# refresh-bio/fqsqueezer

Measured on AMD Instinct MI355X. Metric: Mbases/s compressed (DNA stream, SE sorted), higher is better.
Workload: dtype u64; 1 GPU; 1000000x150bp SE, G=7500000 (seed 2+rank), -om s -gs 8 -qm n -im n; workers_T=64, blocks=256, per_gpu=one independent file per GPU

## Files before the change

fqsqueezer_amd/csrc/fqsx_api.hip:

```cpp
#include "fqsx_kernels.h"
#include "fqsx_qual.h"
#include "fqsx_qdec.h"
#include "../../include/fqsx.h"
#include "fqsx_vm.h"
#include "fqsx_rt.h"
#include <sys/resource.h>

#ifndef FQSX_EMU
#include <dlfcn.h>
#include <rccl/rccl.h>
#endif
#include <algorithm>
#include <cstdio>
#include <cstdlib>
#include <cstring>
#include <string>
#include <vector>

extern "C" const char *fqsx_last_error(void) { return g_err.c_str(); }
extern "C" const char *fqsx_version(void) {
#ifdef FQSX_EMU
  return "fqsx 0.1 (host emulation build - tests only)";
#else
  return "fqsx 0.1 (HIP gfx950)";
#endif
}

FQ_DEV bool phase_skip(const DevCfg &cfg) { return (cfg.err[0] | cfg.err[1]) != 0; }
FQ_KERNEL_NW(FQSX_INS_THREADS, FQSX_INS_WG_PER_CU * FQSX_INS_WAVES / 4) void k_insert_phase(DevCfg cfg, u64 nb_slots, u64 ns_slots, u32 win, u32 maxmult) {
  FQ_SHARED InsWgShared sm;
#ifndef FQSX_EMU
  if (FQ_TID == 0) sm.err = phase_skip(cfg) ? 1u : 0u;
  __syncthreads();
  const bool skip = sm.err != 0;
  __syncthreads();
  if (skip) return;
#else
  if (phase_skip(cfg)) return;
#endif
  if (FQ_BLOCK >= 3 * cfg.T) {
    const u64 stride = (u64)(FQ_NBLOCKS - 3 * cfg.T) * FQ_NTHREADS, first = (u64)(FQ_BLOCK - 3 * cfg.T) * FQ_NTHREADS + FQ_TID;
    for (u64 i = first; i < nb_slots; i += stride) cfg.l_b.slots[i] = 0;
    for (u64 i = first; i < ns_slots; i += stride) cfg.l_s.slots[i] = 0;
    for (u64 i = first; i < 2ull * cfg.T; i += stride) cfg.l_s.filled[i] = 0;
    return;
  }
  insert_phase_body(cfg, &sm, FQ_BLOCK / 3, FQ_BLOCK % 3, win, maxmult);
  if (cfg.sys_scope) fq_release_system();
}
FQ_KERNEL64 void k_compact_generic(const u8 *out, u64 out_cap, const u64 *lens, u8 *dst) {
  const u32 tid = FQ_BLOCK;
  u64 off = 0;
  for (u32 t = 0; t < tid; ++t) off += lens[t];
  const u64 n = lens[tid] <= out_cap ? lens[tid] : 0;
  const u8 *src = out + (u64)tid * out_cap;
  for (u64 i = FQ_LANE; i < n; i += FQ_WAVE) dst[off + i] = src[i];
}
FQ_KERNEL64 void k_clear_local(DevCfg cfg, u64 nb_slots, u64 ns_slots) {
  if (phase_skip(cfg)) return;
  const u64 stride = (u64)FQ_NBLOCKS * FQ_WAVE, first = (u64)FQ_BLOCK * FQ_WAVE + FQ_LANE;
  for (u64 i = first; i < nb_slots; i += stride) cfg.l_b.slots[i] = 0;
  for (u64 i = first; i < ns_slots; i += stride) cfg.l_s.slots[i] = 0;
  for (u64 i = first; i < 2ull * cfg.T; i += stride) cfg.l_s.filled[i] = 0;
}
FQ_KERNEL64 void k_finish_block(DevCfg cfg, u64 *lens , u64 *end ) {
  if (FQ_LANE == 0) {
    if (FQ_BLOCK == 0) { end[2 * cfg.T] = cfg.err[0]; end[2 * cfg.T + 1] = cfg.err[1]; }
    if (cfg.err[1]) return;
    finish_block_body(cfg, FQ_BLOCK);
    lens[FQ_BLOCK] = cfg.ws[FQ_BLOCK].out_len;
    end[FQ_BLOCK] = cfg.ws[FQ_BLOCK].out_len;
    end[cfg.T + FQ_BLOCK] = cfg.ctx_filled[FQ_BLOCK];
  }
}
FQ_KERNEL64 void k_gather_stats(DevCfg cfg, u64 *out) {
  for (u32 i = FQ_LANE; i < 64; i += FQ_WAVE) {
    u64 s = 0;
    for (u32 t = 0; t < cfg.T; ++t) s += cfg.ws[t].stat[i];
    out[i] = s;
  }
}
FQ_DEV void part_split(const DevCfg &cfg, u32 &kind, u32 &blk) {
  kind = 0;
  blk = FQ_BLOCK;
  for (; kind < 2; ++kind) {
    const u32 g = cfg.T * cfg.mail[kind].n_tiles;
    if (blk < g) break;
    blk -= g;
  }
}
FQ_KERNEL64 void k_part_count(DevCfg cfg) {
  FQ_SHARED u32 hist[256];
  u32 kind, blk;
  if (phase_skip(cfg)) return;
  part_split(cfg, kind, blk);
  part_count_body(cfg, kind, blk, hist);
}
FQ_KERNEL64 void k_part_scan(DevCfg cfg) {
  if (phase_skip(cfg)) return;
  part_scan_body(cfg, FQ_BLOCK / cfg.T, FQ_BLOCK % cfg.T);
}
FQ_DEV void part_dstoff_leader(const DevCfg &cfg, u32 kind, u32 *demand , u32 seg1);
FQ_KERNEL64 void k_part_dstoff(DevCfg cfg, u32 *demand , u32 seg1) {
  if (cfg.err[0] || (cfg.err[1] && cfg.err[1] != seg1)) {
    if (FQ_BLOCK == 0 && FQ_LANE == 0) demand[2 * cfg.T] = cfg.err[0];
    return;
  }
  part_dstoff_leader(cfg, FQ_BLOCK, demand, seg1);
}
FQ_DEV void part_dstoff_leader(const DevCfg &cfg, u32 kind, u32 *demand, u32 seg1) {
  part_dstoff_body(cfg, kind);
  if (kind != MAIL_P)
    for (u32 d = FQ_LANE; d < cfg.T; d += FQ_WAVE) {
      const u32 o = (kind == MAIL_S ? 0 : cfg.T) + d;
      demand[o] = cfg.mail[kind].dst_tot[d];
      demand[2 * cfg.T + 1 + o] = (kind == MAIL_S ? cfg.g_s : cfg.g_b).filled[d];
    }
  if (kind == 0 && FQ_LANE == 0) demand[2 * cfg.T] = *cfg.err;
  if (seg1 && kind != MAIL_P) {
    const KTab &t = kind == MAIL_S ? cfg.g_s : cfg.g_b;
    bool over = false;
    for (u32 d = FQ_LANE; d < cfg.T; d += FQ_WAVE) over |= ((u64)t.filled[d] + cfg.mail[kind].dst_tot[d]) * 100 > t.nb * FQSX_BKT * cfg.tab_load_pct;
    if (wave_any(over) && FQ_LANE == 0) cfg.err[1] = seg1;
  }
}
FQ_KERNEL64 void k_part_scatter(DevCfg cfg, u32 seg1, u32 *demand) {
  FQ_SHARED u32 cursor[256];
  FQ_SHARED u32 ld[64];
  FQ_SHARED u64 gm[256];
  FQ_SHARED u32 doff[257];
  u32 kind, blk;
  if (cfg.err[0] || (cfg.err[1] && cfg.err[1] != seg1)) return;
  part_split(cfg, kind, blk);
  if (demand) {
    const Mail &m = cfg.mail[kind];
    u32 run = 0;
    for (u32 base = 0; base < cfg.T; base += FQ_WAVE) {
      const u32 d = base + FQ_LANE;
      const u32 v = d < cfg.T ? m.dst_tot[d] : 0;
      const u32 ex = wave_excl_scan32(v) + run;
      if (d < cfg.T) doff[d] = ex;
      run += wave_sum32(v);
    }
    if (FQ_LANE == 0) doff[cfg.T] = run;
    FQ_SYNC();
    if (blk == 0) part_dstoff_leader(cfg, kind, demand, seg1);
  }
  part_scatter_body(cfg, kind, blk, cursor, ld, gm, demand ? doff : nullptr);
}
FQ_KERNEL64 void k_pe_demand(DevCfg cfg, u32 *demand, u32 seg1) {
  FQ_SHARED InsShared sm;
  if (seg1 && phase_skip(cfg)) return;
  pe_insert_body(cfg, &sm, FQ_BLOCK, true, demand);
  if (seg1 && FQ_LANE == 0 && ((u64)cfg.g_pe.filled[FQ_BLOCK] + demand[FQ_BLOCK]) * 2 > cfg.g_pe.cap_mask + 1) cfg.err[1] = seg1;
}
FQ_KERNEL void k_pe_bucket_count(DevCfg cfg) {
  if (phase_skip(cfg)) return;
  const u32 total = cfg.T * cfg.pe_cap, stride = FQ_GRID_STRIDE(u32);
  for (u32 g = FQ_GRID_FIRST(u32); g < total; g += stride) pe_bucket_count_body(cfg, g);
}
FQ_KERNEL64 void k_pe_bucket_offsets(DevCfg cfg, u32 seg1) {
  if (phase_skip(cfg)) return;
  u32 run = 0;
  bool over = false;
  for (u32 base = 0; base < cfg.T; base += FQ_WAVE) {
    const u32 o = base + FQ_LANE;
    const u32 v = o < cfg.T ? cfg.pe_bkt_n[o] : 0u;
    const u32 ex = wave_excl_scan32(v) + run;
    if (o < cfg.T) {
      cfg.pe_bkt_n[cfg.T + o] = ex;
      cfg.pe_bkt_cur[o] = 0;
      over |= ((u64)cfg.g_pe.filled[o] + v) * 2 > cfg.g_pe.cap_mask + 1;
    }
    run += wave_sum32(v);
  }
  if (FQ_LANE == 0) cfg.pe_bkt_n[2 * cfg.T] = run;
  if (wave_any(over) && FQ_LANE == 0) cfg.err[1] = seg1;
}
FQ_KERNEL void k_pe_bucket_scatter(DevCfg cfg) {
  if (phase_skip(cfg)) return;
  const u32 total = cfg.T * cfg.pe_cap, stride = FQ_GRID_STRIDE(u32);
  for (u32 g = FQ_GRID_FIRST(u32); g < total; g += stride) pe_bucket_scatter_body(cfg, g);
}
FQ_KERNEL64 void k_pe_insert_buckets(DevCfg cfg) {
  FQ_SHARED InsShared sm;
  if (phase_skip(cfg)) return;
  pe_insert_bucket_body(cfg, &sm, FQ_BLOCK);
  FQ_SYNC_MEM();
  if (FQ_LANE == 0) cfg.pe_bkt_n[FQ_BLOCK] = 0;
}
FQ_KERNEL64 void k_pe_insert(DevCfg cfg) {
  FQ_SHARED InsShared sm;
  if (phase_skip(cfg)) return;
  if (cfg.pe_part && FQ_BLOCK % cfg.shard_world != cfg.shard_rank) return;
  pe_insert_body(cfg, &sm, FQ_BLOCK, false, nullptr);
  if (cfg.sys_scope) fq_release_system();
}
FQ_KERNEL void k_rehash_ptab(PTab o, PTab n, u32 n_sub, u32 first, u32 step, u32 sys) {
  const u64 ocap = o.cap_mask + 1, total = ocap * n_sub;
  const u64 gstride = FQ_GRID_STRIDE(u64);
  for (u64 g = FQ_GRID_FIRST(u64); g < total; g += gstride) {
    const u32 sub = first + (u32)(g / ocap) * step;
    const u64 k = o.key[(u64)sub * o.stride + (g % ocap)], v = o.val[(u64)sub * o.stride + (g % ocap)];
    if (k == 0 && v == 0) continue;
    u64 *nk = n.key + (u64)sub * n.stride, *nv = n.val + (u64)sub * n.stride;
    u64 p = murmur64(k) & n.cap_mask;
    for (;;) {
      if (nk[p] == 0 && atomic_cas64(&nk[p], 0, k) == 0) { nv[p] = v; break; }
      p = (p + 1) & n.cap_mask;
    }
  }
  if (sys) fq_release_system();
}
FQ_KERNEL void k_zero_words(u64 *p, u64 n, u32 sys) {
  const u64 gstride = FQ_GRID_STRIDE(u64);
  for (u64 i = FQ_GRID_FIRST(u64); i < n; i += gstride) p[i] = 0;
  if (sys) fq_release_system();
}
FQ_KERNEL void k_rehash_ktab(KTab o, KTab n, u32 n_sub, u32 first, u32 step, u32 sys) {
  const u64 ocap = o.nb * FQSX_BKT;
  const u64 total = ocap * n_sub;
  const u64 gstride = FQ_GRID_STRIDE(u64);
  for (u64 g = FQ_GRID_FIRST(u64); g < total; g += gstride) {
    u32 sub = first + (u32)(g / ocap) * step;
    u64 it = o.slots[(u64)sub * o.stride + (g % ocap)];
    if (!it) continue;
    bool claimed = false;
    (void)tab_find_or_claim(n, n.slots + (u64)sub * n.stride, it >> n.cbits, it, claimed);
  }
  if (sys) fq_release_system();
}
FQ_KERNEL void k_rehash_ctx(const u64 *o, u64 ocap_mask, u64 *n, u64 ncap_mask, u32 T) {
  const u64 ocap = ocap_mask + 1, total = ocap * T;
  const u64 gstride = FQ_GRID_STRIDE(u64);
  for (u64 g = FQ_GRID_FIRST(u64); g < total; g += gstride) {
    u32 w = (u32)(g / ocap);
    const u64 *src = o + 4 * g;
    u64 q1 = src[1];
    u32 tag = slot_tag(q1);
    if (!tag) continue;
    u64 key = src[0];
    u64 *b = n + 4 * (u64)w * (ncap_mask + 1);
    u64 h = (u64)ctx_mix(tag, key) & ncap_mask;
    for (;;) {
      u64 *p = b + 4 * h;
      if (p[1] == 0 && atomic_cas64(&p[1], 0, q1) == 0) {
        p[0] = key; p[2] = src[2]; p[3] = src[3];
        break;
      }
      h = (h + 1) & ncap_mask;
    }
  }
}

FQ_KERNEL64 void k_shard_counts(DevCfg cfg, u32 *dst, u32 status) {
  const u32 T = cfg.T;
  if (FQ_BLOCK == 3 * T) {
    for (u32 s = FQ_LANE; s < T; s += FQ_WAVE) dst[3ull * T * T + s] = (cfg.pe_n && shard_mine(cfg, s)) ? cfg.pe_n[s] : 0u;
    if (FQ_LANE == 0) dst[3ull * T * T + T] = (status | cfg.err[0]) != 0 ? 1u : 0u;
    return;
  }
  const u32 kind = FQ_BLOCK / T, s = FQ_BLOCK % T;
  const Mail &m = cfg.mail[kind];
  for (u32 o = FQ_LANE; o < T; o += FQ_WAVE) {
    u32 n = 0;
    if (shard_mine(cfg, s))
      for (u32 t = 0; t < m.n_tiles; ++t) n += m.tile_hist[((u64)s * m.n_tiles + t) * T + cfg.vmap[o]];
    dst[((u64)kind * T + s) * T + o] = n;
  }
}
FQ_KERNEL void k_shard_colsum(DevCfg cfg, const u32 *C, u32 *cs) {
  const u32 T = cfg.T, G = cfg.shard_world;
  const u32 stride = FQ_GRID_STRIDE(u32), first = FQ_GRID_FIRST(u32);
  for (u32 i = first; i < 3 * T; i += stride) {
    const u32 kind = i / T, o = i % T;
    const u32 *Ck = C + (u64)kind * T * T;
    u32 tot = 0;
    for (u32 q = 0; q < G; ++q) {
      u32 n = 0;
      for (u32 s = q; s < T; s += 8 * G) {
        u32 v[8];
#pragma unroll
        for (u32 x = 0; x < 8; ++x) v[x] = s + x * G < T ? Ck[(u64)(s + x * G) * T + o] : 0u;
#pragma unroll
        for (u32 x = 0; x < 8; ++x) n += v[x];
      }
      cs[((u64)kind * (G + 1) + 1 + q) * T + o] = n;
      tot += n;
    }
    cs[((u64)kind * (G + 1)) * T + o] = tot;
  }
}
FQ_KERNEL64 void k_shard_need(DevCfg cfg, const u32 *cs, u64 *out, u64 *stats_before) {
  const u32 T = cfg.T;
  for (u32 which = 0; which < 2; ++which) {
    const KTab &t = which ? cfg.g_b : cfg.g_s;
    const u32 *tot = cs + (u64)(which ? MAIL_B : MAIL_S) * (cfg.shard_world + 1) * T;
    u64 need = 0;
    for (u32 o = FQ_LANE; o < T; o += FQ_WAVE) {
      const u64 n = (u64)t.filled[o] + tot[o];
      need = n > need ? n : need;
// ... 88 lines not shown
    if (o == T - 1) m.dst_off[T] = dst + tot;
  }
  if (o % G != me) return;
  u32 run = 0;
  for (u32 sb = 0; sb < T; sb += FQ_WAVE) {
    const u32 s = sb + FQ_LANE;
    const u32 v = s < T ? Ck[(u64)s * T + o] : 0u;
    const u32 ex = wave_excl_scan32(v) + run;
    if (s < T) { col[s] = v; pre[s] = ex; }
    run += wave_sum32(v);
  }
  FQ_SYNC();
  u32 chunk0 = 0;
  for (u32 q = 0; q < G; ++q) {
    u32 before = 0, size = 0;
    for (u32 jb = 0; jb < n_own; jb += FQ_WAVE) {
      const u32 j = jb + FQ_LANE, o2 = me + j * G;
      u32 n = 0;
      if (j < n_own) {
        if (cs) n = cs[((u64)kind * (G + 1) + 1 + q) * T + o2];
        else for (u32 s = q; s < T; s += G) n += Ck[(u64)s * T + o2];
      }
      before += wave_sum32(j < n_own && o2 < o ? n : 0u);
      size += wave_sum32(j < n_own ? n : 0u);
    }
    u32 src = chunk0 + before;
    for (u32 s = q; s < T; s += G) {
      if (FQ_LANE == 0) soff[s] = src;
      src += col[s];
    }
    chunk0 += size;
  }
  FQ_SYNC();
  for (u32 x = FQ_LANE; x < tot; x += FQ_WAVE) {
    u32 lo = 0, hi = T;
    while (hi - lo > 1) {
      const u32 mid = (lo + hi) >> 1;
      if (pre[mid] <= x) lo = mid; else hi = mid;
    }
    while (col[lo] == 0 && lo > 0) --lo;
    m.sorted[dst + x] = recv[soff[lo] + (x - pre[lo])];
  }
}
FQ_KERNEL void k_shard_collect(DevCfg cfg, u32 kind, u64 *out) {
  const Mail &m = cfg.mail[kind];
  const u32 total = m.dst_off[cfg.T];
  const u32 stride = FQ_GRID_STRIDE(u32), first = FQ_GRID_FIRST(u32);
  for (u32 e = first; e < total; e += stride) {
    const u64 x = m.sorted[e];
    if (kind == MAIL_P) { out[e] = (x << 2) | siv_test(&cfg, x); continue; }
    const KTab &t = kind == MAIL_S ? cfg.g_s : cfg.g_b;
    const u64 *sl = t.slots + (u64)sb_owner(&cfg, x) * t.stride;
    const u64 item = tab_locate(t, sl, x >> (64 - 2 * t.k)).item;
    out[e] = item;
  }
}
FQ_KERNEL void k_shard_apply(DevCfg cfg, u32 kind, const u64 *items, u32 n) {
  const u32 stride = FQ_GRID_STRIDE(u32), first = FQ_GRID_FIRST(u32);
  for (u32 e = first; e < n; e += stride) {
    const u64 item = items[e];
    if (kind == MAIL_P && cfg.siv_part) {
      if (item) siv_idx_move(cfg, item >> 4, (u32)((item >> 2) & 3), (u32)(item & 3));
      continue;
    }
    if (kind == MAIL_P) {
      const u64 idx = item >> 2, val = item & 3;
      u64 *wp = cfg.siv + (idx >> 5);
      const u32 sh = 2 * (u32)(idx & 31);
      u64 old = *wp;
      for (;;) {
        if (((old >> sh) & 3) >= val) break;
        const u64 seen = atomic_cas64(wp, old, (old & ~(3ull << sh)) | (val << sh));
        if (seen == old) { siv_idx_move(cfg, idx, (u32)((old >> sh) & 3), (u32)val); break; }
        old = seen;
      }
      continue;
    }
    if (!item) continue;
    const KTab &t = kind == MAIL_S ? cfg.g_s : cfg.g_b;
    const u64 v = item >> t.cbits;
    const u32 sub = sb_owner(&cfg, v << (64 - 2 * t.k));
    bool claimed = false;
    u64 *slot = tab_find_or_claim(t, t.slots + (u64)sub * t.stride, v, item, claimed);
    if (!slot) continue;
    if (claimed) {
      atomic_add32(&t.filled[sub], 1u);
      continue;
    }
    u64 old = *(volatile u64 *)slot;
    while ((old & ((1ull << t.cbits) - 1ull)) < (item & ((1ull << t.cbits) - 1ull))) {
      const u64 seen = atomic_cas64(slot, old, item);
      if (seen == old) break;
      old = seen;
    }
  }
}

struct fqsx_dna : DevCtx {
  DevCfg cfg;
  u32 T;
  u64 gs_cap, gb_cap, ls_cap, lb_cap, ctx_cap, gpe_cap, lpe_cap;
  u32 pe_bkt_cap;
  bool paired;
  u32 mail_cap[3];
  u64 dev_bases_cap, dev_off_cap;
  u8 *d_bases;
  u64 *d_off;
  u32 *d_demand;
  u64 *d_lens;
  u8 *d_compact;
  u64 compact_cap, din_cap, dout_cap;
  std::vector<u32> h_demand, h_filled;
  std::vector<u8> h_out;
  std::vector<u64> h_lens;
  u32 n_growths;
  u32 tab_small_pct;
  u32 tab_load_pct, tab_after_pct;
  u8 *h_pin;
  u64 *d_end;
  bool filled_valid;
  u32 cur_n_reads, cur_S, cur_gen;
  u64 cur_need_lb, cur_need_ls, cur_need_lpe;
  bool cur_decode;
  u32 shard_rank, shard_world = 1;
  u8 *d_vmap;
  u64 *d_xbuf;
  u64 xbuf_cap;
  u32 *d_cglob;
  u32 *d_colsum;
  u64 siv_before[2];
  fqsx_comm comm;
  bool comm_set, shard_apply_own;
  u64 *d_xrecv[3];
  u64 xrecv_cap[3];
  u64 *d_items, *d_gathered, *d_small;
  u64 items_cap, gathered_cap;
  std::vector<u32> h_cglob;
  u64 sh_phases, sh_collectives, sh_a2a_words, sh_gather_words;
  bool part;
  bool part_fallback;
  u64 vm_gran;
  fqsx_vm::FdMesh mesh;
  struct VmTab {
    u8 *va = nullptr;
    u64 va_bytes = 0, chunk_bytes = 0;
    std::vector<fqsx_vm::Handle> h;
    std::vector<u8> mapped;
    u64 own_bytes = 0;
    u32 own_mod = 0;
    bool live = false;
  } vm_s, vm_b, vm_pk, vm_pv, vm_siv;
  u32 *d_plog_n;
  u32 ins_win, ins_maxmult;
  u64 vm_own_bytes;
};

namespace {

#define FQSX_PIN_BYTES (64u * 1024u)
int d2h_small_begin(fqsx_dna *c, const void *d, u64 bytes) { return d2h(c, c->h_pin, d, bytes); }
int d2h_small_end(fqsx_dna *c, void *h, u64 bytes) {
  DEVCHK(dev_sync(c));
  memcpy(h, c->h_pin, bytes);
  return FQSX_OK;
}

#define REHASH_GRID FQ_GRID(2048)

int collect_streams(DevCtx *c, u8 *d_compact, u32 T, const u8 *d_out, u64 out_cap, const u64 *d_lens,
                    const std::vector<u64> &lens_host, std::vector<u8> &h_out, const u8 **streams, u64 *lens) {
  int rc;
  u64 total = 0;
  for (u32 t = 0; t < T; ++t) total += lens_host[t];
  h_out.resize(total ? total : 1);
  if (total) {
    LAUNCH(c, 2, k_compact_generic, T, 64, d_out, out_cap, d_lens, d_compact);
    if ((rc = d2h_sync(c, h_out.data(), d_compact, total))) return rc;
  }
  u64 pos = 0;
  for (u32 t = 0; t < T; ++t) {
    streams[t] = h_out.data() + pos;
    lens[t] = lens_host[t];
    pos += lens_host[t];
  }
  return FQSX_OK;
}

u64 pow2_at_least(u64 x) {
  u64 p = 1;
  while (p < x) p <<= 1;
  return p;
}

bool tab_over(const fqsx_dna *c, u64 need, u64 cap) { return need * 100 > cap * c->tab_load_pct; }
u64 tab_new_cap(const fqsx_dna *c, u64 need) {
  const u32 after = need * c->T * sizeof(u64) * 100 / 40 < (256ull << 20) ? std::min<u32>(c->tab_small_pct, c->tab_after_pct) : c->tab_after_pct;
  u64 cap = (need * 100 + after - 1) / after + 2 * FQSX_BKT;
  return (cap + FQSX_BKT - 1) / FQSX_BKT * FQSX_BKT;
}

KGeom make_geom(u32 k) {
  KGeom g;
  g.k = k;
  g.shift = 64 - 2 * k;
  g.mask = (~0ull) << g.shift;
  g.kernel_mask = ((1ull << (2 * k - 8)) - 1ull) << (64 - 2 * k + 4);
  return g;
}

void mt_seed(u32 *s, u32 seed) {
  s[0] = seed;
  for (int i = 1; i < 624; ++i) s[i] = 1812433253u * (s[i - 1] ^ (s[i - 1] >> 30)) + (u32)i;
}

int ktab_alloc(fqsx_dna *c, KTab &t, u32 n_sub, u64 cap, u32 k, u32 cbits, bool with_filled) {
  void *p = nullptr;
  int rc = dalloc(c, &p, cap * n_sub * sizeof(u64), true);
  if (rc) return rc;
  t.slots = (u64 *)p;
  t.nb = cap / FQSX_BKT;
  t.stride = cap;
  t.k = k;
  t.cbits = cbits;
  if (with_filled) {
    rc = dalloc(c, &p, (u64)n_sub * sizeof(u32), true);
    if (rc) return rc;
    t.filled = (u32 *)p;
  }
  return FQSX_OK;
}

#define VMCHK(x) do { std::string e_; if (g_vm_dbg) fprintf(stderr, "[fqsx vm] %s\n", #x); if ((x)) { g_err = "partitioned tables: " + e_; return FQSX_E_HIP; } } while (0)
static const bool g_vm_dbg = getenv("FQSX_VM_DEBUG") != nullptr;
u32 vt_rank(const fqsx_dna *c, const fqsx_dna::VmTab &v, u32 o) { return (v.own_mod ? o % v.own_mod : o) % c->shard_world; }
void vtab_drop(fqsx_dna *c, fqsx_dna::VmTab &v, u32 o) {
  if (!v.live || !v.mapped[o]) return;
  std::string e;
  (void)fqsx_vm::unmap(v.va + (u64)o * v.chunk_bytes, v.chunk_bytes, e);
  (void)fqsx_vm::release(v.h[o], e);
  v.mapped[o] = 0;
  if (vt_rank(c, v, o) == c->shard_rank) { c->dev_bytes -= v.chunk_bytes; c->vm_own_bytes -= v.chunk_bytes; v.own_bytes -= v.chunk_bytes; }
}
void vtab_free(fqsx_dna *c, fqsx_dna::VmTab &v) {
  if (!v.live) return;
  std::string e;
  for (u32 o = 0; o < (u32)v.h.size(); ++o) vtab_drop(c, v, o);
#ifdef FQSX_EMU
  (void)fqsx_vm::unreserve(v.va, v.va_bytes, e);
#else
#endif
  v = fqsx_dna::VmTab();
}
u64 vm_min_chunk(const fqsx_dna *c) {
#ifndef FQSX_EMU
  return std::max<u64>(c->vm_gran, 2ull << 20);
#else
  return c->vm_gran;
#endif
}
int vtab_reserve_raw(fqsx_dna *c, fqsx_dna::VmTab &v, u64 cap, u64 *stride_out, u32 n_chunks = 0) {
  const u32 T = n_chunks ? n_chunks : c->T;
  const u64 min_chunk = vm_min_chunk(c);
  const u64 gran_slots = min_chunk / sizeof(u64);
  const u64 stride = (cap + gran_slots - 1) / gran_slots * gran_slots;
  v = fqsx_dna::VmTab();
  v.chunk_bytes = stride * sizeof(u64);
  v.va_bytes = v.chunk_bytes * T;
  v.h.assign(T, fqsx_vm::Handle());
  v.mapped.assign(T, 0);
  VMCHK(fqsx_vm::reserve(v.va_bytes, std::max<u64>(c->vm_gran, std::min<u64>(v.chunk_bytes, 2ull << 20)), &v.va, e_));
  v.live = true;
  *stride_out = stride;
  return FQSX_OK;
}
int vtab_reserve(fqsx_dna *c, KTab &t, fqsx_dna::VmTab &v, u64 cap, u32 k, u32 cbits) {
  u64 stride = 0;
  const int rc = vtab_reserve_raw(c, v, cap, &stride);
  if (rc) return rc;
  t.slots = (u64 *)v.va;
  t.nb = cap / FQSX_BKT;
  t.stride = stride;
  t.k = k;
  t.cbits = cbits;
  return FQSX_OK;
}
int vtab_create_own(fqsx_dna *c, fqsx_dna::VmTab &v, u32 o) {
  VMCHK(fqsx_vm::create(c->device, v.chunk_bytes, &v.h[o], e_));
  c->dev_bytes += v.chunk_bytes; c->vm_own_bytes += v.chunk_bytes; v.own_bytes += v.chunk_bytes;
  c->dev_bytes_peak = std::max(c->dev_bytes_peak, c->dev_bytes);
  VMCHK(fqsx_vm::map(c->device, v.va + (u64)o * v.chunk_bytes, v.chunk_bytes, v.h[o], e_));
  v.mapped[o] = 1;
  const u64 words = v.chunk_bytes / sizeof(u64);
  LAUNCH(c, 2, k_zero_words, (u32)std::min<u64>(REHASH_GRID, (words + 255) / 256), 256, (u64 *)(v.va + (u64)o * v.chunk_bytes), words, c->cfg.sys_scope);
  return FQSX_OK;
}
int vtab_exchange(fqsx_dna *c, fqsx_dna::VmTab &v) {
  const u32 T = (u32)v.h.size(), G = c->shard_world, me = c->shard_rank;
  if (G == 1) return FQSX_OK;
  std::vector<std::vector<u32>> of(G);
  for (u32 o = 0; o < T; ++o) of[vt_rank(c, v, o)].push_back(o);
  size_t longest = 0;
  for (u32 q = 0; q < G; ++q) longest = std::max(longest, of[q].size());
  const size_t R = 128;
  for (size_t r0 = 0; r0 < longest; r0 += R) {
    std::vector<int> mine;
    for (size_t j = r0; j < std::min(of[me].size(), r0 + R); ++j) {
// ... 158 lines not shown
  c->n_growths += 1;
  return FQSX_OK;
}

int grow_ctx(fqsx_dna *c, u64 new_cap) {
  void *p = nullptr;
  int rc = dalloc(c, &p, new_cap * c->T * sizeof(CtxSlot), true);
  if (rc) return rc;
  LAUNCH(c, 2, k_rehash_ctx, REHASH_GRID, 256, (const u64 *)c->cfg.ctx, c->cfg.ctx_cap_mask, (u64 *)p, new_cap - 1, c->T);
  DEVCHK(dev_sync(c));
  dfree(c, c->cfg.ctx);
  c->cfg.ctx = (CtxSlot *)p;
  c->cfg.ctx_cap_mask = new_cap - 1;
  c->ctx_cap = new_cap;
  return FQSX_OK;
}

int mail_alloc(fqsx_dna *c, u32 kind, u32 cap) {
  Mail &m = c->cfg.mail[kind];
  const u32 T = c->T;
  dfree(c, m.list); dfree(c, m.sorted); dfree(c, m.tile_hist);
  m.list = m.sorted = nullptr; m.tile_hist = nullptr;
  m.cap = m.n_tiles = 0; c->mail_cap[kind] = 0;
  cap = (cap + FQSX_TILE - 1) / FQSX_TILE * FQSX_TILE;
  void *p = nullptr;
  int rc;
  if ((rc = dalloc(c, &p, (u64)T * cap * sizeof(u64), false))) return rc;
  m.list = (u64 *)p;
  if ((rc = dalloc(c, &p, (u64)T * cap * sizeof(u64), false))) return rc;
  m.sorted = (u64 *)p;
  m.cap = cap;
  m.n_tiles = cap / FQSX_TILE;
  if ((rc = dalloc(c, &p, (u64)T * m.n_tiles * T * sizeof(u32), false))) return rc;
  m.tile_hist = (u32 *)p;
  c->mail_cap[kind] = cap;
  return FQSX_OK;
}

int launch_segment(fqsx_dna *c, bool decode, u32 n_reads, u32 S, u32 seg) {
  EncArgs a;
  a.cfg = c->cfg;
  a.n_reads = n_reads; a.S = S; a.seg = seg; a.pad = (u32)c->k_n[0];
  return dev_launch(c, 0, true, [&] {
    return decode ? fqsx_launch_decode(c->stream, a) : c->paired ? fqsx_launch_encode_pe(c->stream, a) : fqsx_launch_encode_se(c->stream, a);
  });
}

int block_prepare(fqsx_dna *c, const u8 *d_bases, const u64 *d_off, const u64 *h_off, u32 n_reads, u32 generation,
                  const u8 *const *dec_streams = nullptr, const u64 *dec_lens = nullptr) {
  const bool decode = dec_streams != nullptr;
  const u32 T = c->T;
  DevCfg &cfg = c->cfg;
  u64 S = generation < 100u ? 100u - generation : 0u;
  u64 cap_s = (u64)n_reads / T / 2;
  if (S > cap_s) S = cap_s;
  if (S) --S;
  u64 max_wbases = 0, max_seg_bases = 0, max_seg_reads = 0, max_wreads = 0;
  std::vector<u64> wbases(T);
  for (u32 t = 0; t < T; ++t) {
    u64 first, last;
    worker_reads(t, T, n_reads, first, last);
    wbases[t] = h_off[last] - h_off[first];
    max_wbases = std::max(max_wbases, wbases[t]);
    max_wreads = std::max(max_wreads, last - first);
    u64 cur = first;
    for (u64 seg = 0; seg <= S; ++seg) {
      u64 stop = last;
      if (seg < S) {
        const u64 ns = segment_synchro(seg, S, first, last);
        if (!c->paired) stop = ns + 1;
        else { u64 i = cur; if (i < ns) i += (ns - i + 1) & ~1ull; stop = i + 2; }
      }
      if (stop > last) stop = last;
      if (stop > cur) {
        max_seg_bases = std::max(max_seg_bases, h_off[stop] - h_off[cur]);
        max_seg_reads = std::max(max_seg_reads, stop - cur);
        cur = stop;
      }
    }
  }
  int rc;
  void *p = nullptr;
  if (c->paired && (n_reads & 1)) { g_err = "paired-end blocks need an even number of reads"; return FQSX_E_ARG; }
  u64 need_out = max_wbases + 16 * max_wreads + 1024;
  if ((rc = dfit(c, cfg.out, cfg.out_cap, need_out, pow2_at_least(need_out), T))) return rc;
  const u64 mail_entries[3] = {2 * max_seg_bases + 2 * max_seg_reads, max_seg_bases, 2 * max_seg_bases};
  for (u32 k = 0; k < 3; ++k) {
    u64 need = mail_entries[k] + 64;
    if (need > c->mail_cap[k] && (rc = mail_alloc(c, k, (u32)(need + need / 4)))) return rc;
  }
  u64 need_lb = pow2_at_least(4 * max_seg_bases + 64), need_ls = pow2_at_least(2 * max_seg_bases + 64);
  if ((rc = ltab_fit(c, cfg.l_b, c->lb_cap, need_lb, cfg.bmer, 6))) return rc;
  if ((rc = ltab_fit(c, cfg.l_s, c->ls_cap, need_ls, cfg.smer, 12))) return rc;
  u64 need_lpe = 0;
  if (c->paired) {
    const u64 seg_pairs = max_seg_reads / 2 + 1;
    const u64 need_list = 14 * seg_pairs + 16;
    const u32 list_cap = (u32)(need_list + need_list / 4);
    if ((rc = dfit(c, cfg.pe_bkt, c->pe_bkt_cap, need_list, list_cap, (u64)T * 3 * sizeof(u64)))) return rc;
    if ((rc = dfit(c, cfg.pe_list, cfg.pe_cap, need_list, list_cap, (u64)T * 3 * sizeof(u64)))) return rc;
    need_lpe = pow2_at_least(2 * 14 * seg_pairs + 64);
    if ((rc = lpe_fit(c, cfg.l_pe, c->lpe_cap, need_lpe))) return rc;
    cfg.l_pe.cap_mask = need_lpe - 1;
    cfg.l_pe.stride = need_lpe;
    u64 max_len = 0;
    for (u32 i = 0; i < n_reads; ++i) max_len = std::max(max_len, h_off[i + 1] - h_off[i]);
    if (!decode && max_len > FQSX_RD_LDS && (rc = dfit(c, cfg.pe_scr, cfg.pe_scr_cap, max_len + 128, (max_len + max_len / 4 + 128 + 63) & ~63ull, (u64)T * 3, true))) return rc;
  }
  cfg.l_b.nb = need_lb / FQSX_BKT; cfg.l_b.stride = need_lb;
  cfg.l_s.nb = need_ls / FQSX_BKT; cfg.l_s.stride = need_ls;
  if (!c->filled_valid && (rc = d2h_sync(c, c->h_filled.data(), cfg.ctx_filled, T * sizeof(u32)))) return rc;
  c->filled_valid = false;
  {
    u64 need = 0;
    for (u32 t = 0; t < T; ++t) need = std::max<u64>(need, (u64)c->h_filled[t] + 2 * wbases[t] + 64);
#ifdef FQSX_TIMING
    if (generation % 64 == 63) fprintf(stderr, "[timing] block %u: ctx slots used by worker 0: %u, capacity %llu\n", generation, c->h_filled[0], (unsigned long long)c->ctx_cap);
#endif
    if (need * 2 > c->ctx_cap && (rc = grow_ctx(c, pow2_at_least(need * 2)))) return rc;
  }
  cfg.bases = d_bases;
  cfg.read_off = d_off;
  if (decode) {
    std::vector<u64> doff(T + 1, 0);
    for (u32 t = 0; t < T; ++t) doff[t + 1] = doff[t] + dec_lens[t];
    u64 max_len = 0;
    for (u32 i = 0; i < n_reads; ++i) max_len = std::max(max_len, h_off[i + 1] - h_off[i]);
    const u64 need_in = doff[T] + 64, need_out = h_off[n_reads] + 64, need_sc = max_len + 64;
    if ((rc = dfit(c, cfg.din, c->din_cap, need_in, need_in + need_in / 4, 1))) return rc;
    if ((rc = dfit(c, cfg.dout, c->dout_cap, need_out, need_out + need_out / 4, 1))) return rc;
    if ((rc = dfit(c, cfg.dscratch, cfg.dcap, need_sc, need_sc + need_sc / 4, (u64)T * 2))) return rc;
    if (!cfg.din_off && (rc = dalloc(c, &p, ((u64)T + 1) * sizeof(u64), false))) return rc;
    if (!cfg.din_off) cfg.din_off = (const u64 *)p;
    std::vector<u8> flat(doff[T] ? doff[T] : 1);
    for (u32 t = 0; t < T; ++t) memcpy(flat.data() + doff[t], dec_streams[t], dec_lens[t]);
    if ((rc = h2d(c, (void *)cfg.din, flat.data(), doff[T]))) return rc;
    if ((rc = h2d(c, (void *)cfg.din_off, doff.data(), (T + 1) * sizeof(u64)))) return rc;
    DEVCHK(dev_sync(c));
  }

  c->cur_n_reads = n_reads; c->cur_S = (u32)S; c->cur_gen = generation;
  c->cur_need_lb = need_lb; c->cur_need_ls = need_ls; c->cur_need_lpe = need_lpe;
  c->cur_decode = decode;
  return FQSX_OK;
}

int clear_local_tables(fqsx_dna *c) {
  const u64 words = (c->cur_need_lb + c->cur_need_ls) * c->T;
  const u32 grid = (u32)std::min<u64>(2048, (words + 4095) / 4096 + 1);
  LAUNCH(c, 2, k_clear_local, grid, 64, c->cfg, c->cur_need_lb * c->T, c->cur_need_ls * c->T);
  return FQSX_OK;
}

int insert_and_clear(fqsx_dna *c) {
  const u64 words = (c->cur_need_lb + c->cur_need_ls) * c->T;
  const u64 per = 64ull * FQSX_INS_THREADS;
  const u32 cgrid = (u32)std::min<u64>(2048, (words + per - 1) / per + 1);
  LAUNCH(c, 1, k_insert_phase, 3 * c->T + cgrid, FQSX_INS_THREADS, c->cfg, c->cur_need_lb * c->T, c->cur_need_ls * c->T, c->ins_win, c->ins_maxmult);
  return FQSX_OK;
}
int grow_for_demand(fqsx_dna *c) {
  const u32 T = c->T;
  DevCfg &cfg = c->cfg;
  int rc;
  for (int which = 0; which < 2; ++which) {
    KTab &t = which ? cfg.g_b : cfg.g_s;
    u64 &cap = which ? c->gb_cap : c->gs_cap;
    u64 need = 0;
    for (u32 o = 0; o < T; ++o) need = std::max<u64>(need, (u64)c->h_demand[2 * T + 1 + which * T + o] + c->h_demand[which * T + o]);
    if (tab_over(c, need, cap) && (rc = grow_global(c, t, cap, tab_new_cap(c, need)))) return rc;
  }
  return FQSX_OK;
}
int pe_insert_and_clear(fqsx_dna *c);
int pe_clear_local(fqsx_dna *c);
int block_recover(fqsx_dna *c, u32 seg) {
  const u32 T = c->T;
  int rc;
  if ((rc = d2h_sync(c, c->h_demand.data(), c->d_demand, (4 * T + 1) * sizeof(u32)))) return rc;
  const u64 before = c->gs_cap + c->gb_cap + c->gpe_cap;
  if ((rc = grow_for_demand(c))) return rc;
  if ((rc = dzero(c, c->cfg.err + 1, sizeof(u32)))) return rc;
  if (c->paired) {
    if ((rc = dzero(c, c->cfg.pe_bkt_n, T * sizeof(u32)))) return rc;
    LAUNCH(c, 2, k_pe_demand, T, 64, c->cfg, c->d_demand + 4 * T + 1, 0u);
    std::vector<u32> dem(T), fil(T);
    if ((rc = d2h_sync(c, dem.data(), c->d_demand + 4 * T + 1, T * sizeof(u32)))) return rc;
    if ((rc = d2h_sync(c, fil.data(), c->cfg.g_pe.filled, T * sizeof(u32)))) return rc;
    u64 need = 0;
    for (u32 o = 0; o < T; ++o) need = std::max<u64>(need, (u64)fil[o] + dem[o]);
    if (need * 2 > c->gpe_cap && (rc = grow_gpe(c, pow2_at_least(need * 2 + 2)))) return rc;
  }
  if (c->gs_cap + c->gb_cap + c->gpe_cap == before) { g_err = "phase " + std::to_string(seg) + " posted for growth, but no table needs it"; return FQSX_E_DEVICE; }
  if (c->paired && (rc = pe_insert_and_clear(c))) return rc;
  return insert_and_clear(c);
}
int pe_clear_local(fqsx_dna *c) {
  const u32 T = c->T;
  DevCfg &cfg = c->cfg;
  int rc;
  if ((rc = dzero(c, cfg.l_pe.key, c->cur_need_lpe * T * sizeof(u64)))) return rc;
  if ((rc = dzero(c, cfg.l_pe.val, c->cur_need_lpe * T * sizeof(u64)))) return rc;
  return dzero(c, cfg.l_pe.filled, T * sizeof(u32));
}
int pe_insert_and_clear(fqsx_dna *c) {
  LAUNCH(c, 2, k_pe_insert, c->T, 64, c->cfg);
  return pe_clear_local(c);
}

int block_segment(fqsx_dna *c, u32 seg) {
  const u32 T = c->T, n_reads = c->cur_n_reads;
  const u64 S = c->cur_S, need_lpe = c->cur_need_lpe;
  const bool decode = c->cur_decode;
  DevCfg &cfg = c->cfg;
  int rc;
  {
    if ((rc = launch_segment(c, decode, n_reads, (u32)S, seg))) return rc;
    const u32 part_grid = T * (cfg.mail[0].n_tiles + cfg.mail[1].n_tiles + cfg.mail[2].n_tiles);
    LAUNCH(c, 2, k_part_count, part_grid, 64, cfg);
    LAUNCH(c, 2, k_part_scan, 3 * T, 64, cfg);
    if (!decode) {
      LAUNCH(c, 2, k_part_scatter, part_grid, 64, cfg, seg + 1, c->d_demand);
      if (c->paired) {
        const u32 bgrid = FQ_GRID((u32)std::min<u64>(1024, ((u64)T * cfg.pe_cap + 255) / 256));
        LAUNCH(c, 2, k_pe_bucket_count, bgrid, 256, cfg);
        LAUNCH(c, 2, k_pe_bucket_offsets, 1, 64, cfg, seg + 1);
        LAUNCH(c, 2, k_pe_bucket_scatter, bgrid, 256, cfg);
        LAUNCH(c, 2, k_pe_insert_buckets, T, 64, cfg);
        if ((rc = pe_clear_local(c))) return rc;
      }
      return insert_and_clear(c);
    }
    LAUNCH(c, 2, k_part_dstoff, 3, 64, cfg, c->d_demand, 0u);
    if ((rc = d2h_small_begin(c, c->d_demand, (4 * T + 1) * sizeof(u32)))) return rc;
    LAUNCH(c, 2, k_part_scatter, part_grid, 64, cfg, 0u, (u32 *)nullptr);
    if ((rc = d2h_small_end(c, c->h_demand.data(), (4 * T + 1) * sizeof(u32)))) return rc;
    if (c->h_demand[2 * T]) {
      g_err = "device error " + std::to_string(c->h_demand[2 * T]) + " in encode kernel";
      return FQSX_E_DEVICE;
    }
    if ((rc = grow_for_demand(c))) return rc;
    if (c->paired) {
      LAUNCH(c, 2, k_pe_demand, T, 64, cfg, c->d_demand, 0u);
      if ((rc = d2h_sync(c, c->h_demand.data(), c->d_demand, T * sizeof(u32)))) return rc;
      if ((rc = d2h_sync(c, c->h_filled.data(), cfg.g_pe.filled, T * sizeof(u32)))) return rc;
      u64 need = 0;
      for (u32 o = 0; o < T; ++o) need = std::max<u64>(need, (u64)c->h_filled[o] + c->h_demand[o]);
      if (need * 2 > c->gpe_cap && (rc = grow_gpe(c, pow2_at_least(need * 2 + 2)))) return rc;
      if ((rc = pe_insert_and_clear(c))) return rc;
    }
    LAUNCH(c, 1, k_insert_phase, 3 * T, FQSX_INS_THREADS, cfg, (u64)0, (u64)0, c->ins_win, c->ins_maxmult);
    if ((rc = clear_local_tables(c))) return rc;
  }
  return FQSX_OK;
}

int block_finish(fqsx_dna *c, const u64 *h_off, const u8 **streams, u64 *lens, u8 *bases_out, u32 *posted = nullptr) {
  if (posted) *posted = 0;
  const u32 T = c->T, n_reads = c->cur_n_reads, generation = c->cur_gen;
  const bool decode = c->cur_decode;
  DevCfg &cfg = c->cfg;
  int rc;
  if (decode) {
    u32 derr = 0;
    if ((rc = d2h_sync(c, &derr, cfg.err, sizeof(u32)))) return rc;
    if (derr) {
      g_err = "device error " + std::to_string(derr) + " while decoding block " + std::to_string(generation);
      return FQSX_E_DEVICE;
    }
    return bases_out ? d2h_sync(c, bases_out, cfg.dout, h_off[n_reads]) : FQSX_OK;
  }
  LAUNCH(c, 2, k_finish_block, T, 64, cfg, c->d_lens, c->d_end);
  {
    std::vector<u64> e(2 * T + 2);
    if ((rc = d2h_small_begin(c, c->d_end, e.size() * sizeof(u64)))) return rc;
    if ((rc = d2h_small_end(c, e.data(), e.size() * sizeof(u64)))) return rc;
    if (e[2 * T]) {
      g_err = "device error " + std::to_string(e[2 * T]) + " while encoding block " + std::to_string(generation);
      return FQSX_E_DEVICE;
    }
    if (e[2 * T + 1]) {
      if (posted) { *posted = (u32)e[2 * T + 1]; return FQSX_OK; }
      g_err = "growth posted by the device outside the deferred path";
      return FQSX_E_DEVICE;
    }
    for (u32 t = 0; t < T; ++t) { c->h_lens[t] = e[t]; c->h_filled[t] = (u32)e[T + t]; }
    c->filled_valid = true;
  }
  u64 total = 0;
  for (u32 t = 0; t < T; ++t) {
    if (c->h_lens[t] > cfg.out_cap) { g_err = "stream overflow"; return FQSX_E_DEVICE; }
    total += c->h_lens[t];
  }
  if ((rc = dfit(c, c->d_compact, c->compact_cap, total, total + total / 2 + 4096, 1))) return rc;
  return collect_streams(c, c->d_compact, T, cfg.out, cfg.out_cap, c->d_lens, c->h_lens, c->h_out, streams, lens);
}

int encode_block_impl(fqsx_dna *c, const u8 *d_bases, const u64 *d_off, const u64 *h_off, u32 n_reads, u32 generation,
                      const u8 **streams, u64 *lens, const u8 *const *dec_streams = nullptr, const u64 *dec_lens = nullptr,
                      u8 *bases_out = nullptr) {
  if (c->shard_world > 1) { g_err = "a sharded codec is driven through fqsx_shard_* (fqsqueezer_amd/sharded.py)"; return FQSX_E_ARG; }
  int rc = block_prepare(c, d_bases, d_off, h_off, n_reads, generation, dec_streams, dec_lens);
  for (u32 seg = 0; !rc;) {
    for (; !rc && seg <= c->cur_S; ++seg) rc = block_segment(c, seg);
    u32 posted = 0;
    if (!rc) rc = block_finish(c, h_off, streams, lens, bases_out, &posted);
    if (rc || !posted) break;
    rc = block_recover(c, posted - 1);
    seg = posted;
  }
  return rc;
}

int create_impl(fqsx_dna *c, const u8 *h) {
  const u32 T = c->T;
  DevCfg &cfg = c->cfg;
  memset(&cfg, 0, sizeof(cfg));
  cfg.T = T;
  cfg.mode = h[5];
  cfg.prefix = h[10]; cfg.pmer = h[11]; cfg.smer = h[12]; cfg.bmer = h[13];
  cfg.gp = make_geom(cfg.pmer); cfg.gs = make_geom(cfg.smer); cfg.gb = make_geom(cfg.bmer);
  cfg.pmer_mod_shift = 2 * cfg.pmer - 12;
  cfg.T_magic = ((1ull << 32) + T - 1) / T;
  cfg.T_pow2 = (T & (T - 1)) == 0 ? 1u : 0u;
  cfg.dbg = 0;
  if (const char *e = getenv("FQSX_PROTO_DEBUG")) cfg.dbg = (u32)strtoul(e, nullptr, 0);
  cfg.ps_nobytes_n = (2 * cfg.pmer + 7) / 8;
  int rc;
  void *p = nullptr;
  if ((rc = dalloc(c, &p, (1ull << (2 * cfg.pmer)) / 4, true))) return rc;
  cfg.siv = (u64 *)p;
  if ((rc = dalloc(c, &p, 2 * sizeof(u64), true))) return rc;
  cfg.siv_stats = (u64 *)p;
  if ((rc = dalloc(c, &p, ((1ull << (2 * cfg.pmer)) >> FQSX_SIV_BLK_LOG) * 4 * sizeof(u32), true))) return rc;
  cfg.siv_idx = (u32 *)p;
  c->tab_load_pct = 80; c->tab_after_pct = 62;
  if (const char *e = getenv("FQSX_TAB_LOAD_PCT")) c->tab_load_pct = (u32)std::min<u64>(85, std::max<u64>(20, strtoull(e, nullptr, 10)));
  c->tab_small_pct = 40;
  if (const char *e = getenv("FQSX_TAB_AFTER_PCT")) c->tab_small_pct = c->tab_after_pct = (u32)std::min<u64>(c->tab_load_pct - 5, std::max<u64>(10, strtoull(e, nullptr, 10)));
  cfg.tab_load_pct = c->tab_load_pct;
  c->ins_win = FQSX_WIN_MAX; c->ins_maxmult = 16;
  if (const char *e = getenv("FQSX_INS_WINDOW")) c->ins_win = (u32)std::min<u64>(FQSX_WIN_MAX, std::max<u64>(1, strtoull(e, nullptr, 10)));
  if (const char *e = getenv("FQSX_INS_MAXMULT")) c->ins_maxmult = (u32)std::min<u64>(FQSX_WIN_MULT_MAX, std::max<u64>(1, strtoull(e, nullptr, 10)));
  if (const char *e = getenv("FQSX_INS_PARALLEL")) if (atoi(e) == 0) c->ins_win = 0;
#ifdef FQSX_EMU
  c->ins_win = 0;
#endif
  if (const char *e = getenv("FQSX_WHATIF")) { u32 r = 0, u = 0; if (sscanf(e, "%u,%u", &r, &u) == 2) cfg.whatif = (r << 16) | (u & 0xffffu); }
  c->gs_cap = c->gb_cap = pow2_at_least(std::max<u64>(1024, (1ull << 22) / T));
  if (const char *e = getenv("FQSX_GTAB_INIT")) c->gs_cap = c->gb_cap = pow2_at_least(std::max<u64>(64, strtoull(e, nullptr, 10)));
  if ((rc = ktab_alloc(c, cfg.g_s, T, c->gs_cap, cfg.smer, 12, true))) return rc;
  if ((rc = ktab_alloc(c, cfg.g_b, T, c->gb_cap, cfg.bmer, 6, true))) return rc;
  cfg.g_s.two = cfg.g_b.two = 1;
  c->ls_cap = c->lb_cap = 1024;
  if ((rc = ktab_alloc(c, cfg.l_s, T, c->ls_cap, cfg.smer, 12, false))) return rc;
  if ((rc = ktab_alloc(c, cfg.l_b, T, c->lb_cap, cfg.bmer, 6, false))) return rc;
  if ((rc = dalloc(c, &p, 2 * (u64)T * sizeof(u32), true))) return rc;
  cfg.l_s.filled = (u32 *)p;
  cfg.l_b.filled = (u32 *)p + T;
  c->ctx_cap = 1u << 14;
  if ((rc = dalloc(c, &p, c->ctx_cap * T * sizeof(CtxSlot), true))) return rc;
  cfg.ctx = (CtxSlot *)p;
  cfg.ctx_cap_mask = c->ctx_cap - 1;
  if ((rc = dalloc(c, &p, T * sizeof(u32), true))) return rc;
  cfg.ctx_filled = (u32 *)p;
  {
    std::vector<u16> tpl(SM_OFF_BYTE, 0);
    auto fill = [&](u32 off, u32 entries, u32 stride, u32 n) {
      for (u32 e = 0; e < entries; ++e) {
        for (u32 i = 0; i < n; ++i) tpl[off + e * stride + i] = 1;
        tpl[off + e * stride + n] = (u16)n;
      }
    };
    fill(SM_OFF_FLAGS, 256, SM_FLAGS_N + 1, SM_FLAGS_N);
    fill(SM_OFF_NS, 32, SM_NS_N + 1, SM_NS_N);
    fill(SM_OFF_PSF, 65536, SM_PSF_N + 1, SM_PSF_N);
    fill(SM_OFF_PSNB, 65536, 6, cfg.ps_nobytes_n);
    fill(SM_OFF_NIB, 68, SM_NIB_N + 1, SM_NIB_N);
    tpl.resize(SM_TOTAL_U16, 0);
    fill(SM_OFF_MID, 1, SM_NIB_N + 1, SM_NIB_N);
    if ((rc = dalloc(c, &p, (u64)T * SM_TOTAL_U16 * sizeof(u16), false))) return rc;
    cfg.small = (u16 *)p;
    if ((rc = h2d(c, cfg.small, tpl.data(), tpl.size() * sizeof(u16)))) return rc;
    DEVCHK(dev_sync(c));
    for (u32 t = 1; t < T; ++t)
      if ((rc = d2d(c, cfg.small + (u64)t * SM_TOTAL_U16, cfg.small, tpl.size() * sizeof(u16)))) return rc;
    if ((rc = dalloc(c, &p, (u64)T * SM_LAZY_ENTRIES, true))) return rc;
    cfg.byte_init = (u8 *)p;
  }
  {
    std::vector<WState> ws(1);
    memset(ws.data(), 0, sizeof(WState));
    for (int g = 0; g < 4; ++g) {
      mt_seed(ws[0].mt[g], 5481);
      ws[0].mt_idx[g] = 624;
    }
    if ((rc = dalloc(c, &p, (u64)T * sizeof(WState), false))) return rc;
    cfg.ws = (WState *)p;
    for (u32 t = 0; t < T; ++t)
      if ((rc = h2d(c, cfg.ws + t, ws.data(), sizeof(WState)))) return rc;
    DEVCHK(dev_sync(c));
  }
  for (u32 k = 0; k < 3; ++k) {
    if ((rc = dalloc(c, &p, (u64)T * sizeof(u32), true))) return rc;
    cfg.mail[k].n = (u32 *)p;
    if ((rc = dalloc(c, &p, (u64)T * sizeof(u32), true))) return rc;
    cfg.mail[k].dst_tot = (u32 *)p;
    if ((rc = dalloc(c, &p, ((u64)T + 1) * sizeof(u32), true))) return rc;
    cfg.mail[k].dst_off = (u32 *)p;
    if ((rc = mail_alloc(c, k, FQSX_TILE))) return rc;
  }
  c->paired = cfg.mode >= 2;
  c->gpe_cap = c->lpe_cap = 0;
  if (c->paired) {
    c->gpe_cap = pow2_at_least(std::max<u64>(1024, (1ull << 20) / T));
    if (const char *e = getenv("FQSX_PTAB_INIT")) c->gpe_cap = pow2_at_least(std::max<u64>(64, strtoull(e, nullptr, 10)));
    if ((rc = ptab_alloc(c, cfg.g_pe, T, c->gpe_cap, true))) return rc;
    c->lpe_cap = 1024;
    if ((rc = ptab_alloc(c, cfg.l_pe, T, c->lpe_cap, true))) return rc;
    if ((rc = dalloc(c, &p, (u64)T * sizeof(u32), true))) return rc;
    cfg.pe_n = (u32 *)p;
    if ((rc = dalloc(c, &p, (3 * (u64)T + 1) * sizeof(u32), true))) return rc;
    cfg.pe_bkt_n = (u32 *)p;
    cfg.pe_bkt_cur = cfg.pe_bkt_n + 2 * T + 1;
  }
  {
    u8 ident[256];
    for (u32 i = 0; i < 256; ++i) ident[i] = (u8)i;
    if ((rc = dalloc(c, &p, 256, false))) return rc;
    c->d_vmap = (u8 *)p;
    cfg.vmap = c->d_vmap;
    if ((rc = h2d(c, c->d_vmap, ident, 256))) return rc;
    DEVCHK(dev_sync(c));
  }
  cfg.shard_rank = 0; cfg.shard_world = 1; cfg.shard_cnt = nullptr;
  if ((rc = dalloc(c, &p, sizeof(u32) * 4, true))) return rc;
  cfg.err = (u32 *)p;
#ifdef FQSX_TIMING
  if ((rc = dalloc(c, &p, (u64)FQSX_TRACE_LAUNCHES * T * FQSX_TRACE_W * sizeof(u64), true))) return rc;
  cfg.trace = (u64 *)p;
#endif
  if ((rc = dalloc(c, &p, (5 * (u64)T + 2) * sizeof(u32), true))) return rc;
  c->d_demand = (u32 *)p;
  if ((rc = dalloc(c, &p, ((u64)T + 64) * sizeof(u64), true))) return rc;
  c->d_lens = (u64 *)p;
  if ((rc = dalloc(c, &p, (2 * (u64)T + 2) * sizeof(u64), true))) return rc;
  c->d_end = (u64 *)p;
  if ((rc = pinned_alloc((void **)&c->h_pin, FQSX_PIN_BYTES))) return rc;
  c->h_demand.assign(4 * T + 1, 0);
  c->h_filled.assign(T, 0);
  c->h_lens.assign(T + 64, 0);
  DEVCHK(dev_sync(c));
  return FQSX_OK;
}

}

extern "C" {

int fqsx_dna_create(const uint8_t *h, int device, fqsx_dna **out) { return fqsx_dna_create_on_partition(h, device, 0, 1, out); }

int fqsx_dna_create_on_partition(const uint8_t *h, int device, uint32_t part, uint32_t n_parts, fqsx_dna **out) {
  if (n_parts == 0 || part >= n_parts) { g_err = "bad compute-unit partition"; return FQSX_E_ARG; }
  if (!h || !out || h[0] != 'K' || h[1] != 'C' || h[2] != 'S' || h[3] != 'D') {
    g_err = "malformed .fqs parameter header";
    return FQSX_E_ARG;
  }
  if (h[4] == 0) { g_err = "no_threads must be >= 1"; return FQSX_E_ARG; }
  if (h[5] > 3) { g_err = "unknown dna_mode"; return FQSX_E_ARG; }
  if (h[11] < 12 || h[11] > 18 || h[12] <= h[11] || h[13] <= h[12] + 1 || h[13] > 27 || h[10] >= h[11]) {
    g_err = "unsupported k-mer lengths";
    return FQSX_E_ARG;
  }
  fqsx_dna *c = new fqsx_dna();
  c->T = h[4];
  int rc = dev_open(c, device, part, n_parts);
  if (rc) {
    delete c;
    return rc;
  }
  rc = create_impl(c, h);
  if (!rc && getenv("FQSX_CHUNKED_TABLES") && atoi(getenv("FQSX_CHUNKED_TABLES"))) rc = fqsx_dna_use_chunked_tables(c);
  if (rc) {
    fqsx_dna_destroy(c);
    return rc;
  }
  *out = c;
  return FQSX_OK;
}

void fqsx_dna_destroy(fqsx_dna *c) {
  if (!c) return;
  dev_close(c);
  vtab_free(c, c->vm_s);
  vtab_free(c, c->vm_b);
  vtab_free(c, c->vm_pk);
  vtab_free(c, c->vm_pv);
  vtab_free(c, c->vm_siv);
  fqsx_vm::mesh_close(c->mesh);
  pinned_free(c->h_pin);
  delete c;
}

int fqsx_dna_encode_block_dev(fqsx_dna *c, const uint8_t *d_bases, const uint64_t *d_off, const uint64_t *h_off,
                              uint32_t n_reads, uint32_t generation, const uint8_t **streams, uint64_t *lens) {
  if (!c || !d_bases || !d_off || !h_off || !streams || !lens) { g_err = "null argument"; return FQSX_E_ARG; }
  DEVCHK(dev_enter(c));
  return encode_block_impl(c, d_bases, d_off, h_off, n_reads, generation, streams, lens);
}

int fqsx_dna_encode_block(fqsx_dna *c, const uint8_t *bases, const uint64_t *off, uint32_t n_reads, uint32_t generation,
                          const uint8_t **streams, uint64_t *lens) {
  if (!c || !bases || !off || !streams || !lens) { g_err = "null argument"; return FQSX_E_ARG; }
  DEVCHK(dev_enter(c));
  int rc;
  u64 nb = off[n_reads] + 64, no = ((u64)n_reads + 1) * sizeof(u64);
  if ((rc = dfit(c, c->d_bases, c->dev_bases_cap, nb, nb + nb / 4, 1))) return rc;
  if ((rc = dfit(c, c->d_off, c->dev_off_cap, no, no + no / 4, 1))) return rc;
  if ((rc = h2d(c, c->d_bases, bases, off[n_reads]))) return rc;
  if ((rc = h2d(c, c->d_off, off, no))) return rc;
  return encode_block_impl(c, c->d_bases, c->d_off, off, n_reads, generation, streams, lens);
}

int fqsx_dna_decode_block(fqsx_dna *c, const uint8_t *const *streams, const uint64_t *lens, const uint64_t *off, uint32_t n_reads,
                          uint32_t generation, uint8_t *bases_out) {
  if (!c || !streams || !lens || !off || !bases_out) { g_err = "null argument"; return FQSX_E_ARG; }
  DEVCHK(dev_enter(c));
  int rc;
  u64 no = ((u64)n_reads + 1) * sizeof(u64);
  if ((rc = dfit(c, c->d_off, c->dev_off_cap, no, no + no / 4, 1))) return rc;
  if ((rc = h2d(c, c->d_off, off, no))) return rc;
  return encode_block_impl(c, nullptr, c->d_off, off, n_reads, generation, nullptr, nullptr, streams, lens, bases_out);
}

int fqsx_dna_decode_block_dev(fqsx_dna *c, const uint8_t *const *streams, const uint64_t *lens, const uint64_t *off, uint32_t n_reads,
                              uint32_t generation, const uint8_t **d_bases_out) {
  if (d_bases_out) *d_bases_out = nullptr;
  if (!c || !streams || !lens || !off || !d_bases_out) { g_err = "null argument"; return FQSX_E_ARG; }
  DEVCHK(dev_enter(c));
  int rc;
  u64 no = ((u64)n_reads + 1) * sizeof(u64);
  if ((rc = dfit(c, c->d_off, c->dev_off_cap, no, no + no / 4, 1))) return rc;
  if ((rc = h2d(c, c->d_off, off, no))) return rc;
  if ((rc = encode_block_impl(c, nullptr, c->d_off, off, n_reads, generation, nullptr, nullptr, streams, lens, nullptr))) return rc;
  *d_bases_out = c->cfg.dout;
  return FQSX_OK;
}

int fqsx_shard_config(fqsx_dna *c, uint32_t rank, uint32_t world) {
  if (!c || world == 0 || rank >= world || world > c->T) { g_err = "bad rank / world size"; return FQSX_E_ARG; }
  if (c->part && world > 1) { g_err = "a codec with chunked tables cannot be sharded afterwards (fqsx_shard_partition_tables after the attach)"; return FQSX_E_ARG; }
  DEVCHK(dev_enter(c));
  const u32 T = c->T;
  c->shard_rank = rank; c->shard_world = world;
  c->cfg.shard_rank = rank; c->cfg.shard_world = world;
  u8 vm[256];
  for (u32 i = 0; i < 256; ++i) vm[i] = (u8)i;
  u32 v = 0;
  for (u32 q = 0; q < world; ++q)
    for (u32 o = q; o < T; o += world) vm[o] = (u8)v++;
  int rc;
  void *p = nullptr;
  if ((rc = h2d(c, c->d_vmap, vm, 256))) return rc;
  if (!c->cfg.shard_cnt) {
    if ((rc = dalloc(c, &p, (3ull * T * T + T + 1) * sizeof(u32), true))) return rc;
    c->cfg.shard_cnt = (u32 *)p;
    if ((rc = dalloc(c, &p, (3ull * T * T + T + 1) * sizeof(u32), true))) return rc;
    c->d_cglob = (u32 *)p;
    if ((rc = dalloc(c, &p, 3ull * (T + 1) * T * sizeof(u32), true))) return rc;
    c->d_colsum = (u32 *)p;
    if ((rc = dalloc(c, &p, 8 * sizeof(u64), true))) return rc;
    c->d_small = (u64 *)p;
    c->h_cglob.assign(3ull * T * T + T + 1, 0);
  }
  DEVCHK(dev_sync(c));
  return FQSX_OK;
}

int fqsx_shard_begin_block(fqsx_dna *c, const uint8_t *bases , const uint64_t *off , const uint64_t *h_off,
                           uint32_t n_reads, uint32_t generation, uint32_t *n_segments) {
  if (!c || !bases || !off || !h_off || !n_segments) { g_err = "null argument"; return FQSX_E_ARG; }
  if (c->part) { g_err = "partitioned tables are driven through fqsx_shard_encode_block"; return FQSX_E_ARG; }
  if (c->paired && c->shard_world > 1) { g_err = "paired-end files are sharded through fqsx_shard_attach + fqsx_shard_encode_block (the step-wise fqsx_shard_* driver does not exchange the pair-table triples)"; return FQSX_E_ARG; }
  DEVCHK(dev_enter(c));
  int rc = block_prepare(c, bases, off, h_off, n_reads, generation);
  *n_segments = c->cur_S + 1;
  return rc;
}

int fqsx_shard_encode(fqsx_dna *c, uint32_t seg, uint32_t *counts ) {
  if (!c || !counts) { g_err = "null argument"; return FQSX_E_ARG; }
  DEVCHK(dev_enter(c));
  const u32 T = c->T;
  DevCfg &cfg = c->cfg;
  int rc;
  if ((rc = launch_segment(c, false, c->cur_n_reads, c->cur_S, seg))) return rc;
  const u32 part_grid = T * (cfg.mail[0].n_tiles + cfg.mail[1].n_tiles + cfg.mail[2].n_tiles);
  LAUNCH(c, 2, k_part_count, part_grid, 64, cfg);
  LAUNCH(c, 2, k_shard_counts, 3 * T + 1, 64, cfg, cfg.shard_cnt, 0u);
  if ((rc = d2d(c, counts, cfg.shard_cnt, 3ull * T * T * sizeof(u32)))) return rc;
  u32 err = 0;
  if ((rc = d2h_sync(c, &err, cfg.err, sizeof(u32)))) return rc;
  if (err) { g_err = "device error " + std::to_string(err) + " in encode kernel"; return FQSX_E_DEVICE; }
  return FQSX_OK;
}

int fqsx_shard_pack(fqsx_dna *c, const uint32_t *counts_sum , uint64_t *const send[3] ) {
  if (!c || !counts_sum || !send) { g_err = "null argument"; return FQSX_E_ARG; }
  DEVCHK(dev_enter(c));
  const u32 T = c->T;
  DevCfg &cfg = c->cfg;
  int rc;
  if ((rc = d2d(c, c->d_cglob, counts_sum, 3ull * T * T * sizeof(u32)))) return rc;
  const u32 part_grid = T * (cfg.mail[0].n_tiles + cfg.mail[1].n_tiles + cfg.mail[2].n_tiles);
  LAUNCH(c, 2, k_part_scan, 3 * T, 64, cfg);
  LAUNCH(c, 2, k_part_dstoff, 3, 64, cfg, c->d_demand, 0u);
  LAUNCH(c, 2, k_part_scatter, part_grid, 64, cfg, 0u, (u32 *)nullptr);
  std::vector<u32> tot(3 * (T + 1));
  for (u32 k = 0; k < 3; ++k)
    if ((rc = d2h_sync(c, tot.data() + k * (T + 1), cfg.mail[k].dst_off, (T + 1) * sizeof(u32)))) return rc;
  for (u32 k = 0; k < 3; ++k) {
    const u64 n = tot[k * (T + 1) + T];
    if (n && (rc = d2d(c, send[k], cfg.mail[k].sorted, n * sizeof(u64)))) return rc;
  }
  DEVCHK(dev_sync(c));
  return FQSX_OK;
}

int fqsx_shard_merge(fqsx_dna *c, const uint64_t *const recv[3] , uint64_t need[2]) {
  if (!c || !recv || !need) { g_err = "null argument"; return FQSX_E_ARG; }
  DEVCHK(dev_enter(c));
  const u32 T = c->T;
  DevCfg &cfg = c->cfg;
  int rc;
  for (u32 k = 0; k < 3; ++k) LAUNCH(c, 2, k_shard_merge, T, 64, cfg, k, recv[k], (const u32 *)c->d_cglob);
  need[0] = need[1] = 0;
  std::vector<u32> tot(T), fil(T);
  for (int which = 0; which < 2; ++which) {
    const KTab &t = which ? cfg.g_b : cfg.g_s;
    if ((rc = d2h_sync(c, tot.data(), cfg.mail[which ? MAIL_B : MAIL_S].dst_tot, T * sizeof(u32)))) return rc;
    if ((rc = d2h_sync(c, fil.data(), t.filled, T * sizeof(u32)))) return rc;
    for (u32 o = 0; o < T; ++o) need[which] = std::max<u64>(need[which], (u64)tot[o] + fil[o]);
  }
  return FQSX_OK;
}

int fqsx_shard_insert(fqsx_dna *c, uint64_t need_s, uint64_t need_b, uint64_t *const items[3] , uint64_t siv_delta[2]) {
  if (!c || !items || !siv_delta) { g_err = "null argument"; return FQSX_E_ARG; }
  DEVCHK(dev_enter(c));
  const u32 T = c->T;
  DevCfg &cfg = c->cfg;
  int rc;
  if (tab_over(c, need_s, c->gs_cap) && (rc = grow_global(c, cfg.g_s, c->gs_cap, tab_new_cap(c, need_s)))) return rc;
  if (tab_over(c, need_b, c->gb_cap) && (rc = grow_global(c, cfg.g_b, c->gb_cap, tab_new_cap(c, need_b)))) return rc;
  if ((rc = d2h_sync(c, c->siv_before, cfg.siv_stats, 2 * sizeof(u64)))) return rc;
  LAUNCH(c, 1, k_insert_phase, 3 * T, FQSX_INS_THREADS, cfg, (u64)0, (u64)0, c->ins_win, c->ins_maxmult);
  u64 after[2];
  if ((rc = d2h_sync(c, after, cfg.siv_stats, 2 * sizeof(u64)))) return rc;
  siv_delta[0] = after[0] - c->siv_before[0];
  siv_delta[1] = after[1] - c->siv_before[1];
  for (u32 k = 0; k < 3; ++k) LAUNCH(c, 2, k_shard_collect, REHASH_GRID, 256, cfg, k, items[k]);
  DEVCHK(dev_sync(c));
  return FQSX_OK;
}

int fqsx_shard_apply(fqsx_dna *c, uint32_t kind, const uint64_t *items , uint64_t n) {
  if (!c || kind > 2 || (!items && n)) { g_err = "bad argument"; return FQSX_E_ARG; }
  DEVCHK(dev_enter(c));
  if (n) LAUNCH(c, 2, k_shard_apply, REHASH_GRID, 256, c->cfg, kind, items, (u32)n);
  return FQSX_OK;
}

int fqsx_shard_end_phase(fqsx_dna *c, const uint64_t siv_delta_sum[2]) {
  if (!c || !siv_delta_sum) { g_err = "null argument"; return FQSX_E_ARG; }
  DEVCHK(dev_enter(c));
  int rc;
  u64 now[2] = {c->siv_before[0] + siv_delta_sum[0], c->siv_before[1] + siv_delta_sum[1]};
  if ((rc = h2d(c, c->cfg.siv_stats, now, 2 * sizeof(u64)))) return rc;
  DEVCHK(dev_sync(c));
  return clear_local_tables(c);
}

int fqsx_shard_finish_block(fqsx_dna *c, const uint64_t *h_off, const uint8_t **streams, uint64_t *lens) {
  if (!c || !h_off || !streams || !lens) { g_err = "null argument"; return FQSX_E_ARG; }
  DEVCHK(dev_enter(c));
  return block_finish(c, h_off, streams, lens, nullptr);
}

namespace {
int xbuf_fit(fqsx_dna *c, u64 *&buf, u64 &cap, u64 words) { return dfit(c, buf, cap, words, words + words / 4 + 1024, sizeof(u64)); }
#define COMMCHK(x, what) do { if ((x) != 0) { if (g_err.empty() || g_err.find(what) == std::string::npos) g_err = std::string(what) + " failed"; if (c->comm.abort) c->comm.abort(c->comm.ctx); return FQSX_E_HIP; } } while (0)

int shard_vote(fqsx_dna *c, int fail, const char *what) {
  const u64 NC = 3ull * c->T * c->T + c->T + 1;
  u32 *word = c->d_cglob + NC - 1;
  u32 v = fail ? 1u : 0u;
  const std::string mine = g_err;
  int rc;
  if ((rc = h2d(c, word, &v, sizeof(v)))) return rc;
  DEVCHK(dev_sync(c));
  COMMCHK(c->comm.allreduce_sum_u32(c->comm.ctx, word, 1), "all-reduce of the phase's status vote");
  if ((rc = d2h_sync(c, &v, word, sizeof(v)))) return rc;
  c->sh_collectives += 1;
  if (fail) { g_err = mine; return fail; }
  if (v) { g_err = std::string("another rank of the world failed in ") + what + " (this rank was fine): the phase is given up on every rank"; return FQSX_E_PEER; }
  return FQSX_OK;
}

int shard_phase_native(fqsx_dna *c, u32 seg) {
  const u32 T = c->T, G = c->shard_world, me = c->shard_rank;
  DevCfg &cfg = c->cfg;
  const u64 NC = 3ull * T * T + T + 1;
  int rc;
  if ((rc = launch_segment(c, false, c->cur_n_reads, c->cur_S, seg))) return rc;
  const u32 part_grid = T * (cfg.mail[0].n_tiles + cfg.mail[1].n_tiles + cfg.mail[2].n_tiles);
  LAUNCH(c, 2, k_part_count, part_grid, 64, cfg);
  LAUNCH(c, 2, k_shard_counts, 3 * T + 1, 64, cfg, c->d_cglob, 0u);
  COMMCHK(c->comm.allreduce_sum_u32(c->comm.ctx, c->d_cglob, NC), "all-reduce of the mailbox counts");
  LAUNCH(c, 2, k_shard_colsum, (3 * T + 63) / 64, 64, cfg, (const u32 *)c->d_cglob, c->d_colsum);
  LAUNCH(c, 2, k_shard_need, 1, 64, cfg, (const u32 *)c->d_colsum, c->d_small + 2, c->d_small);
  u64 small[3];
  if ((rc = d2h(c, c->h_cglob.data(), c->d_cglob, NC * sizeof(u32)))) return rc;
  if ((rc = d2h_sync(c, small, c->d_small + 2, sizeof(small)))) return rc;
  const u32 *C = c->h_cglob.data();
  if (C[NC - 1]) {
    if (small[2]) { g_err = "device error " + std::to_string(small[2]) + " in encode kernel"; return FQSX_E_DEVICE; }
    g_err = "device error in the encode kernel of another rank of the world (this rank was fine): the phase is given up on every rank";
    return FQSX_E_PEER;
  }
  std::vector<u64> vol(3ull * G * G, 0);
  for (u32 k = 0; k < 3; ++k)
    for (u32 s = 0; s < T; ++s)
      for (u32 o = 0; o < T; ++o) vol[((u64)k * G + s % G) * G + o % G] += C[((u64)k * T + s) * T + o];
  LAUNCH(c, 2, k_part_scan, 3 * T, 64, cfg);
  LAUNCH(c, 2, k_part_dstoff, 3, 64, cfg, c->d_demand, 0u);
  LAUNCH(c, 2, k_part_scatter, part_grid, 64, cfg, 0u, (u32 *)nullptr);
  std::vector<u64> sc(3ull * G), rcnt(3ull * G);
  const u64 *send[3];
  u64 *recv[3];
  u64 recv_need[3] = {0, 0, 0};
  for (u32 k = 0; k < 3; ++k) {
    for (u32 q = 0; q < G; ++q) {
      sc[(u64)k * G + q] = vol[((u64)k * G + me) * G + q];
      rcnt[(u64)k * G + q] = vol[((u64)k * G + q) * G + me];
      if (q != me) c->sh_a2a_words += sc[(u64)k * G + q];
      u64 n_in = 0;
      for (u32 f = 0; f < G; ++f) n_in += vol[((u64)k * G + f) * G + q];
      recv_need[k] = std::max(recv_need[k], n_in + 1);
    }
  }
  u64 M[3] = {0, 0, 0}, PM = 0;
  std::vector<u64> n_items(3ull * G, 0), pe_tot(G, 0);
  for (u32 k = 0; k < 3; ++k)
    for (u32 q = 0; q < G; ++q) {
      if (c->part && k != MAIL_P) continue;
      if (G == 1 && !c->shard_apply_own) continue;
      for (u32 f = 0; f < G; ++f) n_items[(u64)k * G + q] += vol[((u64)k * G + f) * G + q];
      M[k] = std::max(M[k], n_items[(u64)k * G + q]);
    }
  const u32 n_own_max = (T + G - 1) / G;
  const u32 n_fill = c->part ? (cfg.pe_part ? 3u : 2u) : 0u;
  const u64 FW = (u64)n_fill * n_own_max;
  if (c->paired)
    for (u32 s = 0; s < T; ++s) { pe_tot[s % G] += C[3ull * T * T + s]; PM = std::max(PM, pe_tot[s % G]); }
  const u64 off_k[3] = {0, M[0], M[0] + M[1]}, off_siv = M[0] + M[1] + M[2], off_fill = off_siv + 2, off_pe = off_fill + FW, W = off_pe + 3 * PM;
  const bool grow_s = tab_over(c, small[0], c->gs_cap), grow_b = tab_over(c, small[1], c->gb_cap);
  int inj_rank = -1, inj_phase = -1;
  if (const char *e = getenv("FQSX_TEST_FAIL")) (void)sscanf(e, "%d,%d", &inj_rank, &inj_phase);
  const bool injected = inj_phase >= 0 && (u64)inj_phase == c->sh_phases;
  if (injected || grow_s || grow_b || W > c->items_cap || W * G > c->gathered_cap || recv_need[0] > c->xrecv_cap[0] || recv_need[1] > c->xrecv_cap[1] ||
      recv_need[2] > c->xrecv_cap[2]) {
    int fail = 0;
    if (injected && (u32)inj_rank == me) { fail = FQSX_E_NOMEM; g_err = "injected allocation failure (FQSX_TEST_FAIL)"; }
    for (u32 k = 0; k < 3 && !fail; ++k) fail = xbuf_fit(c, c->d_xrecv[k], c->xrecv_cap[k], recv_need[k]);
    if (!fail) fail = xbuf_fit(c, c->d_items, c->items_cap, W);
    if (!fail) fail = xbuf_fit(c, c->d_gathered, c->gathered_cap, W * G);
    if (!fail && grow_s) fail = grow_global(c, cfg.g_s, c->gs_cap, tab_new_cap(c, small[0]));
    if (!fail && grow_b) fail = grow_global(c, cfg.g_b, c->gb_cap, tab_new_cap(c, small[1]));
    if (fail && c->part) fqsx_vm::mesh_close(c->mesh);
    if ((rc = shard_vote(c, fail, "the allocations / table growth of a phase"))) return rc;
  }
  for (u32 k = 0; k < 3; ++k) { send[k] = cfg.mail[k].sorted; recv[k] = c->d_xrecv[k]; }
  COMMCHK(c->comm.alltoallv_u64(c->comm.ctx, 3, send, sc.data(), recv, rcnt.data()), "all-to-all of the mailboxes");
  LAUNCH(c, 2, k_shard_merge3, 3 * T, 64, cfg, (const u64 *)c->d_xrecv[0], (const u64 *)c->d_xrecv[1], (const u64 *)c->d_xrecv[2], (const u32 *)c->d_cglob, (const u32 *)c->d_colsum);
  if (cfg.siv_part) {
    cfg.p_log = c->d_items + off_k[MAIL_P];
    if (M[MAIL_P]) LAUNCH(c, 2, k_zero_words, (u32)std::min<u64>(REHASH_GRID, (M[MAIL_P] + 255) / 256), 256, cfg.p_log, M[MAIL_P], 0u);
    if ((rc = dzero(c, c->d_plog_n, sizeof(u32)))) return rc;
  }
  LAUNCH(c, 1, k_insert_phase, 3 * T, FQSX_INS_THREADS, cfg, (u64)0, (u64)0, c->ins_win, c->ins_maxmult);
  for (u32 k = 0; k < 3; ++k)
    if (n_items[(u64)k * G + me] && !(k == MAIL_P && cfg.siv_part)) LAUNCH(c, 2, k_shard_collect, REHASH_GRID, 256, cfg, k, c->d_items + off_k[k]);
  if (FW) LAUNCH(c, 2, k_shard_pack2, 1, 64, cfg, (const u64 *)c->d_small, c->d_items + off_siv, c->d_items + off_fill, n_own_max, n_fill);
  else LAUNCH(c, 2, k_shard_siv_delta, 1, 64, cfg, (const u64 *)c->d_small, c->d_items + off_siv);
  if (c->paired && PM) LAUNCH(c, 2, k_shard_pe_pack, T, 64, cfg, c->d_items + off_pe);
  COMMCHK(c->comm.allgather_u64(c->comm.ctx, c->d_items, W, c->d_gathered), "all-gather of the applied items");
  c->sh_gather_words += W * (G - 1);
  for (u32 q = 0; q < G; ++q)
    if (q != me || c->shard_apply_own)
      for (u32 k = 0; k < 3; ++k)
        if (n_items[(u64)k * G + q] && !(k == MAIL_P && cfg.siv_part && q == me)) LAUNCH(c, 2, k_shard_apply, REHASH_GRID, 256, cfg, k, (const u64 *)(c->d_gathered + (u64)q * W + off_k[k]), (u32)n_items[(u64)k * G + q]);
  if (FW) LAUNCH(c, 2, k_shard_unpack2, 1, 64, cfg, (const u64 *)c->d_small, (const u64 *)c->d_gathered, W, off_siv, off_fill, n_own_max, n_fill);
  else LAUNCH(c, 2, k_shard_siv_sum, 1, 64, cfg, (const u64 *)c->d_small, (const u64 *)c->d_gathered, W, off_siv);
  if (c->paired) {
    if (G > 1 && PM) LAUNCH(c, 2, k_shard_pe_unpack, T, 64, cfg, (const u64 *)c->d_gathered, W, off_pe, (const u32 *)(c->d_cglob + 3ull * T * T));
    LAUNCH(c, 2, k_pe_demand, T, 64, cfg, c->d_demand, 0u);
    if ((rc = d2h_sync(c, c->h_demand.data(), c->d_demand, T * sizeof(u32)))) return rc;
    if ((rc = d2h_sync(c, c->h_filled.data(), cfg.g_pe.filled, T * sizeof(u32)))) return rc;
    u64 need = 0;
    for (u32 o = 0; o < T; ++o) need = std::max<u64>(need, (u64)c->h_filled[o] + c->h_demand[o]);
    if (need * 2 > c->gpe_cap) {
      const int fail = grow_gpe(c, pow2_at_least(need * 2 + 2));
      if (fail && c->part) fqsx_vm::mesh_close(c->mesh);
      if ((rc = shard_vote(c, fail, "the growth of the pair table"))) return rc;
    }
    LAUNCH(c, 2, k_pe_insert, T, 64, cfg);
    if (cfg.pe_part) {
      COMMCHK(c->comm.allreduce_sum_u32(c->comm.ctx, c->d_cglob, 1), "barrier behind the pair-table inserts");
      c->sh_collectives += 1;
    }
    if ((rc = dzero(c, cfg.l_pe.key, c->cur_need_lpe * T * sizeof(u64)))) return rc;
    if ((rc = dzero(c, cfg.l_pe.val, c->cur_need_lpe * T * sizeof(u64)))) return rc;
    if ((rc = dzero(c, cfg.l_pe.filled, T * sizeof(u32)))) return rc;
    c->filled_valid = false;
  }
  c->sh_phases += 1;
  c->sh_collectives += 3;
  return clear_local_tables(c);
}
}

int fqsx_shard_attach(fqsx_dna *c, uint32_t rank, uint32_t world, const fqsx_comm *comm) {
  if (!c || !comm || !comm->allreduce_sum_u32 || !comm->alltoallv_u64 || !comm->allgather_u64) { g_err = "incomplete transport"; return FQSX_E_ARG; }
  int rc = fqsx_shard_config(c, rank, world);
  if (rc) return rc;
  c->comm = *comm;
  c->comm_set = true;
  if (const char *e = getenv("FQSX_SHARD_APPLY_OWN")) c->shard_apply_own = atoi(e) != 0;
  return FQSX_OK;
}

namespace {
int tables_to_chunks(fqsx_dna *c) {
  int rc;
  VMCHK(fqsx_vm::granularity(c->device, &c->vm_gran, e_));
  if (c->vm_gran < sizeof(u64) || (c->vm_gran & (c->vm_gran - 1))) { g_err = "unexpected allocation granularity"; return FQSX_E_HIP; }
  c->part = true;
  c->cfg.sys_scope = (c->shard_world > 1 || (getenv("FQSX_SYS_SCOPE") && atoi(getenv("FQSX_SYS_SCOPE")))) ? 1u : 0u;
  dfree(c, c->cfg.g_s.slots);
  dfree(c, c->cfg.g_b.slots);
  c->cfg.g_s.slots = c->cfg.g_b.slots = nullptr;
  if ((rc = vtab_alloc(c, c->cfg.g_s, c->vm_s, c->gs_cap, c->cfg.smer, 12))) return rc;
  if ((rc = vtab_alloc(c, c->cfg.g_b, c->vm_b, c->gb_cap, c->cfg.bmer, 6))) return rc;
  if (c->paired) {
    dfree(c, c->cfg.g_pe.key);
    dfree(c, c->cfg.g_pe.val);
    c->cfg.g_pe.key = c->cfg.g_pe.val = nullptr;
    if ((rc = ptab_reserve(c, c->cfg.g_pe, c->vm_pk, c->vm_pv, c->gpe_cap))) return rc;
    for (u32 o = c->shard_rank; o < c->T; o += c->shard_world)
      if ((rc = vtab_create_own(c, c->vm_pk, o)) || (rc = vtab_create_own(c, c->vm_pv, o))) return rc;
    if ((rc = vtab_exchange(c, c->vm_pk)) || (rc = vtab_exchange(c, c->vm_pv))) return rc;
    c->cfg.pe_part = c->shard_world > 1 ? 1u : 0u;
  }
  if (c->shard_world > 1 && !(getenv("FQSX_SIV_REPLICA") && atoi(getenv("FQSX_SIV_REPLICA")))) {
    const u64 siv_bytes = (1ull << (2 * c->cfg.pmer)) / 4, range_bytes = siv_bytes / 4096;
    if (range_bytes >= vm_min_chunk(c) && range_bytes % c->vm_gran == 0 && c->cfg.pmer_mod_shift == 2 * c->cfg.pmer - 12) {
      rlimit rl;
      if (getrlimit(RLIMIT_NOFILE, &rl) == 0 && rl.rlim_cur < 16384 && rl.rlim_cur < rl.rlim_max) {
        rl.rlim_cur = std::min<rlim_t>(rl.rlim_max, 16384);
        (void)setrlimit(RLIMIT_NOFILE, &rl);
      }
      dfree(c, c->cfg.siv);
      c->cfg.siv = nullptr;
      u64 stride = 0;
      c->vm_siv = fqsx_dna::VmTab();
      if ((rc = vtab_reserve_raw(c, c->vm_siv, range_bytes / sizeof(u64), &stride, 4096))) return rc;
      if (stride != range_bytes / sizeof(u64)) { g_err = "p-mer vector ranges do not tile the address range"; return FQSX_E_HIP; }
      c->vm_siv.own_mod = c->T;
      for (u32 r = 0; r < 4096; ++r)
        if (vt_rank(c, c->vm_siv, r) == c->shard_rank && (rc = vtab_create_own(c, c->vm_siv, r))) return rc;
      if ((rc = vtab_exchange(c, c->vm_siv))) return rc;
      c->cfg.siv = (u64 *)c->vm_siv.va;
      c->cfg.siv_part = 1;
      void *p = nullptr;
      if ((rc = dalloc(c, &p, 2 * sizeof(u32), true))) return rc;
      c->d_plog_n = (u32 *)p;
      c->cfg.p_log_n = c->d_plog_n;
    }
  }
  DEVCHK(dev_sync(c));
  return FQSX_OK;
}
}

int fqsx_dna_use_chunked_tables(fqsx_dna *c) {
  if (!c) { g_err = "null argument"; return FQSX_E_ARG; }
  if (c->part) return FQSX_OK;
  if (c->k_n[0] || c->shard_world > 1) { g_err = "chunked tables are chosen before the first block (sharded codecs: fqsx_shard_partition_tables)"; return FQSX_E_ARG; }
  DEVCHK(dev_enter(c));
  return tables_to_chunks(c);
}

int fqsx_shard_partition_tables(fqsx_dna *c) {
  if (!c || !c->comm_set) { g_err = "no transport attached (fqsx_shard_attach)"; return FQSX_E_ARG; }
  if (c->part && (c->shard_world == 1 || !c->mesh.peer.empty())) return FQSX_OK;
  if (c->part || c->k_n[0]) { g_err = "the tables can only be partitioned before the first block"; return FQSX_E_ARG; }
  DEVCHK(dev_enter(c));
  const u32 G = c->shard_world, me = c->shard_rank;
  int rc;
  c->part_fallback = false;
#ifndef FQSX_EMU
  if (G > 1) {
    u64 mine[2] = {0, 0};
    char bus[16] = {0};
    HIPCHK(hipDeviceGetPCIBusId(bus, (int)sizeof(bus), c->device));
    memcpy(mine, bus, sizeof(mine));
    std::vector<u64> all(2ull * G, 0);
    if ((rc = xbuf_fit(c, c->d_items, c->items_cap, 2))) return rc;
    if ((rc = xbuf_fit(c, c->d_gathered, c->gathered_cap, 2ull * G))) return rc;
    if ((rc = h2d(c, c->d_items, mine, sizeof(mine)))) return rc;
    DEVCHK(dev_sync(c));
    COMMCHK(c->comm.allgather_u64(c->comm.ctx, c->d_items, 2, c->d_gathered), "all-gather of the ranks' PCI bus ids");
    if ((rc = d2h_sync(c, all.data(), c->d_gathered, all.size() * sizeof(u64)))) return rc;
    std::string why;
    for (u32 q = 0; q < G && why.empty(); ++q) {
      if (q == me) continue;
      char pb[17] = {0};
      memcpy(pb, &all[2ull * q], 16);
      int pd = -1, can = 0;
      if (hipDeviceGetByPCIBusId(&pd, pb) != hipSuccess) { (void)hipGetLastError(); why = std::string("the GPU of rank ") + std::to_string(q) + " (" + pb + ") is not visible to rank " + std::to_string(me); }
      else if (pd != c->device && (hipDeviceCanAccessPeer(&can, c->device, pd) != hipSuccess || !can)) { (void)hipGetLastError(); why = std::string("rank ") + std::to_string(me) + " (" + bus + ") has no peer access to the GPU of rank " + std::to_string(q) + " (" + pb + ")"; }
    }
    u32 v = why.empty() ? 0u : 1u;
    u32 *word = c->d_cglob;
    if ((rc = h2d(c, word, &v, sizeof(v)))) return rc;
    DEVCHK(dev_sync(c));
    COMMCHK(c->comm.allreduce_sum_u32(c->comm.ctx, word, 1), "all-reduce of the peer-access check");
    if ((rc = d2h_sync(c, &v, word, sizeof(v)))) return rc;
    if (v) {
      c->part_fallback = true;
      g_err = "partitioned tables need peer access between all GPUs of the world: " + (why.empty() ? std::string("another rank cannot reach a peer") : why) +
              "; every rank keeps table replicas instead (fqsx_shard_is_partitioned() == 0)";
      return FQSX_OK;
// ... 1529 lines not shown
```

fqsqueezer_amd/csrc/fqsx_dev.h:

```cpp
#pragma once
#include "fqsx_layout.h"
#include "fqsx_rc.h"
#include "fqsx_insplan.h"

#define FQSX_RR 6u
#define FQSX_SW 4u
#define FQSX_NSC 3u
#define FQSX_SCR FQSX_NSC
#define FQSX_RQ 256u
struct SpecBuf {
  u32 h_read, h_i0, h_n;
  u32 h_epoch;
  u32 h_pub;
  u32 h_fix_lane, h_fix_end;
  u32 h_pq_lo[2];
  u32 h_np, h_nlp;
  u64 h_ns, h_nls;
  u64 sp_sdir[6][FQSX_SPEC];
  u64 sp_src[6][FQSX_SPEC];
  u8 sp_scur[6][FQSX_SPEC];
  u64 sp_key[10][FQSX_SPEC];
  u8 sp_kind[FQSX_SPEC];
  u64 sp_cq[FQSX_SPEC];
  u8 sp_lvz[FQSX_SPEC];
// ... 540 lines not shown
FQ_DEV TabLoc tab_locate_as(const KTab &t, const u64 *s, u64 v) {
  TabLoc R;
  R.pos = ~0ull; R.item = 0; R.ns = 0;
  u64 nsl = 0;
  const TabHome h = tab_home(t, v);
  u64 ia[FQSX_BKT];
  tab_load_bucket_as<LIVE>(s, h.a, ia);
  u32 fa, oa;
  bool chain = false;
  if (t.two) {
    u64 ib[FQSX_BKT];
    tab_load_bucket_as<LIVE>(s, h.b, ib);
    u32 fb, ob;
    tab_bucket_find(t, ia, v, fa, oa, nsl);
    tab_bucket_find(t, ib, v, fb, ob, nsl);
    if (fa != FQSX_BKT) { R.item = tab_pick(ia, fa); R.pos = (u64)h.a * FQSX_BKT + fa; }
    else if (fb != FQSX_BKT) { R.item = tab_pick(ib, fb); R.pos = (u64)h.b * FQSX_BKT + fb; }
    else if (oa != FQSX_BKT || ob != FQSX_BKT) R.pos = oa <= ob ? (u64)h.a * FQSX_BKT + oa : (u64)h.b * FQSX_BKT + ob;
    else chain = true;
  } else {
    tab_bucket_find(t, ia, v, fa, oa, nsl);
    if (fa != FQSX_BKT) { R.item = tab_pick(ia, fa); R.pos = (u64)h.a * FQSX_BKT + fa; }
    else if (oa != FQSX_BKT) R.pos = (u64)h.a * FQSX_BKT + oa;
    else chain = true;
  }
  if (chain) {
    u32 p = t.two ? h.b : h.a;
    for (u64 n = 0; n <= t.nb; ++n) {
      p = t.two ? tab_next(t, h.a, p) : ((u64)p + 1 == t.nb ? 0u : p + 1u);
      u64 it[FQSX_BKT];
      tab_load_bucket_as<LIVE>(s, p, it);
      u32 fj, oc;
      tab_bucket_find(t, it, v, fj, oc, nsl);
      if (fj != FQSX_BKT) { R.item = tab_pick(it, fj); R.pos = (u64)p * FQSX_BKT + fj; break; }
      if (oc != FQSX_BKT) { R.pos = (u64)p * FQSX_BKT + oc; break; }
    }
  }
  R.ns = (u32)nsl;
  return R;
}
FQ_DEVN TabLoc tab_locate(const KTab t, const u64 *s, u64 v) { return tab_locate_as<false>(t, s, v); }
FQ_DEVN TabLoc tab_locate_live(const KTab t, const u64 *s, u64 v) { return tab_locate_as<true>(t, s, v); }
FQ_DEV TabLoc tab_locate1(const KTab &t, const u64 *s, u64 v) {
  TabLoc R;
  R.pos = ~0ull; R.item = 0; R.ns = 0;
  u64 nsl = 0;
  u32 p = tab_home(t, v).a;
  for (u64 n = 0; n <= t.nb; ++n) {
    u64 it[FQSX_BKT];
    tab_load_bucket(s, p, it);
    u32 fj, oc;
    tab_bucket_find(t, it, v, fj, oc, nsl);
    if (fj != FQSX_BKT) { R.item = tab_pick(it, fj); R.pos = (u64)p * FQSX_BKT + fj; break; }
    if (oc != FQSX_BKT) { R.pos = (u64)p * FQSX_BKT + oc; break; }
    p = (u64)p + 1 == t.nb ? 0u : p + 1u;
  }
  R.ns = (u32)nsl;
  return R;
}
FQ_DEV u64 *tab_find_or_claim(const KTab &t, u64 *s, u64 v, u64 item, bool &claimed) {
  const TabHome h = tab_home(t, v);
  claimed = false;
  u64 ns_ = 0;
  for (u32 attempt = 0; attempt < 64; ++attempt) {
    u64 ia[FQSX_BKT], ib[FQSX_BKT];
    for (u32 j = 0; j < FQSX_BKT; ++j) ia[j] = ((volatile u64 *)s)[(u64)h.a * FQSX_BKT + j];
    u32 fa, oa, fb = FQSX_BKT, ob = FQSX_BKT;
    tab_bucket_find(t, ia, v, fa, oa, ns_);
    if (fa != FQSX_BKT) return s + (u64)h.a * FQSX_BKT + fa;
    if (t.two) {
      for (u32 j = 0; j < FQSX_BKT; ++j) ib[j] = ((volatile u64 *)s)[(u64)h.b * FQSX_BKT + j];
      tab_bucket_find(t, ib, v, fb, ob, ns_);
      if (fb != FQSX_BKT) return s + (u64)h.b * FQSX_BKT + fb;
    }
    if (oa == FQSX_BKT && ob == FQSX_BKT) break;
    u64 *slot = oa <= ob ? s + (u64)h.a * FQSX_BKT + oa : s + (u64)h.b * FQSX_BKT + ob;
    const u64 seen = atomic_cas64(slot, 0, item);
    if (seen == 0) { claimed = true; return slot; }
    if ((seen >> t.cbits) == v) return slot;
  }
  u32 p = t.two ? h.b : h.a;
  for (u64 n = 0; n <= t.nb; ++n) {
    p = t.two ? tab_next(t, h.a, p) : ((u64)p + 1 == t.nb ? 0u : p + 1u);
    for (u32 j = 0; j < FQSX_BKT; ++j) {
      u64 *slot = s + (u64)p * FQSX_BKT + j;
      u64 it = *(volatile u64 *)slot;
      if (!it) {
        const u64 seen = atomic_cas64(slot, 0, item);
        if (seen == 0) { claimed = true; return slot; }
        it = seen;
      }
      if ((it >> t.cbits) == v) return slot;
    }
  }
  return nullptr;
}
FQ_DEV u32 tab_count(const KTab &t, u32 sub, u64 kmer_norm, u64 &nslots) {
  const TabLoc L = tab_locate(t, t.slots + (u64)sub * t.stride, kmer_norm >> (64 - 2 * t.k));
  nslots += L.ns;
  return (u32)(L.item & ((1ull << t.cbits) - 1ull));
}

FQ_DEV void batch_scan(Wk &w, const KTab &t, bool global, u32 n) {
  WgShared *sm = w.sm;
  u64 ns = 0;
  FQ_SYNC();
  for (u32 i = FQ_LANE; i < n; i += FQ_WAVE) {
    C4 c;
    c4_zero(c);
    u64 key = sm->bk_key[i];
    tab_scan(t, global ? sb_owner(w.cfg, key) : w.tid, key, sm->bk_dir[i] != 0, c, ns);
    sm->bk_res[i][0] = c.c[0];
    sm->bk_res[i][1] = c.c[1];
    sm->bk_res[i][2] = c.c[2];
    sm->bk_res[i][3] = c.c[3];
  }
  FQ_SYNC();
  w.st[global ? ST_GPROBE : ST_LPROBE] += n;
  w.st[global ? ST_GSLOT : ST_LSLOT] += wave_sum64(ns);
}
FQ_DEV void batch_hit_mask(Wk &w, u32 n, u64 mask[4]) {
  WgShared *sm = w.sm;
  mask[0] = mask[1] = mask[2] = mask[3] = 0;
#if FQ_WAVE > 1
  for (u32 r = 0; r * 64 < n; ++r) {
    u32 q = r * 64 + FQ_LANE;
    bool hit = q < n && (sm->bk_res[q][0] | sm->bk_res[q][1] | sm->bk_res[q][2] | sm->bk_res[q][3]) != 0;
    mask[r] = wave_ballot(hit);
  }
#else
  for (u32 q = 0; q < n; ++q)
    if (sm->bk_res[q][0] | sm->bk_res[q][1] | sm->bk_res[q][2] | sm->bk_res[q][3]) mask[q >> 6] |= 1ull << (q & 63);
#endif
}
FQ_DEV void batch_count(Wk &w, const KTab &t, u32 n) {
  WgShared *sm = w.sm;
  u64 ns = 0;
  FQ_SYNC();
  for (u32 i = FQ_LANE; i < n; i += FQ_WAVE) {
    u64 key = sm->bk_key[i];
    sm->bk_res[i][0] = tab_count(t, sb_owner(w.cfg, key), key, ns);
  }
  FQ_SYNC();
  w.st[ST_GPROBE] += n;
  w.st[ST_GSLOT] += wave_sum64(ns);
}

template <class SM>
FQ_DEV void insert_batch(const DevCfg &cfg, SM *sm, const KTab &t, u32 sub, const u64 *keys, u32 n, u32 rng, const Cinc &ci,
                         u64 &nslots, u32 &err);
template <class SM>
FQ_DEV void insert_batch_k(const DevCfg &cfg, SM *sm, const KTab &t, u32 sub, u64 mykey, u32 n, u32 rng, const Cinc &ci,
                           u64 &nslots, u32 &err);
template <class SM>
FQ_DEV void insert_keys(const DevCfg &cfg, SM *sm, const KTab &t, u32 sub, const u64 *keys, u32 n, u32 rng, const Cinc &ci,
                        u64 &nslots, u32 &err) {
#if FQ_WAVE > 1
  const u64 *s = t.slots + (u64)sub * t.stride;
  u64 nextk = FQ_LANE < n ? keys[FQ_LANE] : 0;
  for (u32 o = 0; o < n && !err; o += FQ_WAVE) {
    const u64 k = nextk;
    u64 touch = 0;
    if (o + FQ_WAVE + FQ_LANE < n) {
      nextk = keys[o + FQ_WAVE + FQ_LANE];
      const TabHome th = tab_home(t, nextk >> (64 - 2 * t.k));
      touch = touch_load(&s[(u64)th.a * FQSX_BKT]) ^ touch_load(&s[(u64)th.b * FQSX_BKT]);
    }
    insert_batch_k(cfg, sm, t, sub, k, n - o < FQ_WAVE ? n - o : FQ_WAVE, rng, ci, nslots, err);
    keep_live(touch);
  }
#else
  for (u32 j = 0; j < n && !err; ++j) insert_batch(cfg, sm, t, sub, keys + j, 1, rng, ci, nslots, err);
#endif
}
FQ_DEV u32 lq_done_now(Wk &w, u32 qi) { return w.lqh ? lds_load_acq(&w.sm->lq_done[qi]) : w.la[qi ? MAIL_S : MAIL_B]; }
FQ_DEV void lq_publish(Wk &w, bool force = false) {
  if (!w.lqh) return;
  if (!force && (w.cfg->dbg & FQSX_DBG_INSERTER_STALL)) return;
  const u32 nb = w.mn[MAIL_B], ns = w.mn[MAIL_S];
  if (nb != w.lq_pub[0]) { lds_store_rel(&w.sm->lq_target[0], nb); w.lq_pub[0] = nb; }
  if (ns != w.lq_pub[1]) { lds_store_rel(&w.sm->lq_target[1], ns); w.lq_pub[1] = ns; }
}
FQ_DEV void lq_flush(Wk &w, u32 kind) {
  const Mail &m = w.cfg->mail[kind];
  const u32 qi = kind == MAIL_S ? 1 : 0;
  const u32 n = w.mn[kind];
  if (w.lqh) {
    if (lds_load_acq(&w.sm->lq_done[qi]) >= n) return;
    TM_BEGIN(t_lq);
    TM_COUNT(w, CN_LQFLUSH);
    lq_publish(w, true);
    u32 spins = 0;
    while (lds_load_acq(&w.sm->lq_done[qi]) < n) {
      fq_sleep();
      if (spin_expired(spins)) { w.err = FQSX_ERR_PIPE; break; }
    }
    TM_END(w, TM_LQ, t_lq);
    return;
  }
  const u32 a = w.la[kind];
  if (a >= n) return;
  TM_BEGIN(t_lq);
  TM_COUNT(w, CN_LQFLUSH);
  u64 ns = 0;
  u32 err = 0;
  FQ_SYNC_MEM();
  insert_keys(*w.cfg, w.sm, kind == MAIL_S ? w.cfg->l_s : w.cfg->l_b, w.tid, m.list + (u64)w.tid * m.cap + a, n - a,
              kind == MAIL_S ? RNG_LS : RNG_LB, kind == MAIL_S ? CINC_S : CINC_B, ns, err);
  w.la[kind] = n;
  w.st[ST_LINS] += n - a;
  if (err) w.err = FQSX_ERR_LTAB_FULL;
  TM_END(w, TM_LQ, t_lq);
}
FQ_DEV bool pq_group_hit(Wk &w, u32 qi, const KGeom &g, const Kmer &km, u32 lo, u32 hi) {
  const u32 k2 = 2 * g.k;
  const bool nd = km_norm_dir(km, g);
  const u64 v = (nd ? km.dir : km.rc) >> (64 - k2);
  const u64 lowmask = (1ull << (k2 - 2)) - 1ull;
  const u64 grp = nd ? (v >> 2) : (v & lowmask);
  bool hit = false;
  FQ_SYNC();
  for (u32 t = lo + FQ_LANE; t < hi; t += FQ_WAVE) {
    u64 pv = w.sm->pq_key[qi][t & (FQSX_PQ - 1)] >> (64 - k2);
    hit |= nd ? ((pv >> 2) == grp) : ((pv & lowmask) == grp);
  }
  return wave_any(hit);
}

FQ_DEV void lq_sync_for(Wk &w, u32 kind, const KGeom &g, const Kmer &km) {
  const u32 qi = kind == MAIL_S ? 1 : 0;
  const u32 n = w.mn[kind], d = lq_done_now(w, qi);
  if (d >= n) return;
  bool need = km.cur != g.k || n - d > FQSX_PQ;
  if (!need) need = pq_group_hit(w, qi, g, km, d, n);
  if (need) lq_flush(w, kind);
}

FQ_DEV bool kt_find(Wk &w, const KTab &t, bool global, const KGeom &g, const Kmer &km, u32 rng, const Cinc &ci, C4 &out, u32 pre = 0xff) {
  c4_zero(out);
  if (pre != 0xff) {
    const u32 m = g.k - km.cur, cnt = 1u << (2 * m);
    u64 hm = 0;
    u32 nsl = 0;
    FQ_SYNC();
#if FQ_WAVE > 1
    {
      const bool in = FQ_LANE < cnt;
      const u32 e = pre + (in ? FQ_LANE : 0u);
      hm = wave_ballot(in && w.sb->ep_res[e] != 0);
      nsl = in ? w.sb->ep_ns[e] : 0u;
    }
#else
    for (u32 i = 0; i < cnt; ++i) {
      hm |= (u64)(w.sb->ep_res[pre + i] != 0) << i;
      nsl += w.sb->ep_ns[pre + i];
    }
#endif
    w.st[ST_GPROBE] += cnt;
    w.st[ST_GSLOT] += wave_sum32(nsl);
    if (m == 0) {
      const u64 v = w.sb->ep_res[pre];
      out.c[0] = (u32)(v & 0xffff); out.c[1] = (u32)((v >> 16) & 0xffff); out.c[2] = (u32)((v >> 32) & 0xffff); out.c[3] = (u32)(v >> 48);
      return c4_any(out);
    }
    for (u64 mk = hm; mk; mk &= mk - 1) {
      const u64 v = w.sb->ep_res[pre + ctz64(mk)];
      for (u32 x = 0; x < 4; ++x) {
        const u32 loc = (u32)((v >> (16 * x)) & 0xffff);
        if (loc) out.c[x] = cinc_merge(w.sm, rng, ci, out.c[x], loc);
      }
    }
    return c4_any(out);
  }
  if (km.cur == g.k) {
    u64 ns = 0;
    u64 key = km_norm(km, g);
    tab_scan(t, global ? sb_owner(w.cfg, key) : w.tid, key, km_norm_dir(km, g), out, ns);
    w.st[global ? ST_GPROBE : ST_LPROBE] += 1;
    w.st[global ? ST_GSLOT : ST_LSLOT] += ns;
    return c4_any(out);
  }
  WgShared *sm = w.sm;
  const u32 m = g.k - km.cur;
  const u32 trials = 1u << (2 * m);
  const u64 dir_pad = km.dir >> (2 * m);
  u64 rc_pad = km.rc & (~0ull << (64 - 2 * km.cur));
  for (u32 base = 0; base < trials; base += 256) {
    u32 n = trials - base < 256 ? trials - base : 256;
    FQ_SYNC();
    for (u32 i = FQ_LANE; i < n; i += FQ_WAVE) {
      u32 t_i = base + i;
      u64 d = dir_pad, r = rc_pad;
      for (u32 j = 0; j < m; ++j) {
        u64 sym = (t_i >> (2 * j)) & 3;
        d |= sym << (62 - 2 * j);
        r |= (3 - sym) << (64 - 2 * g.k + 2 * j);
      }
      bool nd = (d & g.kernel_mask) < (r & g.kernel_mask);
      sm->bk_key[i] = nd ? d : r;
      sm->bk_dir[i] = nd ? 1 : 0;
    }
    batch_scan(w, t, global, n);
    u64 hm[4];
    batch_hit_mask(w, n, hm);
    for (u32 r = 0; r < 4; ++r)
      for (u64 mk = hm[r]; mk; mk &= mk - 1) {
        u32 i = r * 64 + ctz64(mk);
        for (u32 s = 0; s < 4; ++s) {
          u32 loc = sm->bk_res[i][s];
          if (loc) out.c[s] = cinc_merge(sm, rng, ci, out.c[s], loc);
        }
      }
  }
  return c4_any(out);
}

FQ_DEV u64 siv_test(const DevCfg *cfg, u64 idx) { return (cfg->siv[idx >> 5] >> (2 * (idx & 31))) & 3; }
FQ_DEV void siv_counts(Wk &w, u64 idx, C4 &c) {
  u64 d = w.cfg->siv[idx >> 5];
  u32 sh = 2 * (u32)((idx & 31) & ~3ull);
  c.c[0] = (u32)((d >> sh) & 3);
  c.c[1] = (u32)((d >> (sh + 2)) & 3);
  c.c[2] = (u32)((d >> (sh + 4)) & 3);
  c.c[3] = (u32)((d >> (sh + 6)) & 3);
  w.st[ST_SIV_WORDS] += 1;
// ... 3093 lines not shown
  w.nsc = MODE >= 2 ? 2u : FQSX_NSC;
  w.rq_p = nullptr; w.rq_size = 0; w.rq_rev = false;
  w.sc_poll = false;
  w.sc_abandoned = false;
  w.sc_read = 0;
  w.sc_epoch = 0;
  w.sc_taken = 0;
  w.sc_base = 0;
  w.rq_early = false;
  w.rq_noscout = false;
  w.cq_head = w.cq_tail = 0;
  w.c_r_sym = 0;
  for (u32 i = 0; i < ST_N; ++i) w.st[i] = 0;
  for (u32 i = 0; i < FQSX_TM_SLOTS; ++i) w.tm[i] = 0;
  TM_BEGIN(t_total);
  TM_STAMP(cfg, tid, launch, 0);
  const u64 T = cfg.T;
  u64 first, last;
  worker_reads(tid, T, n_reads, first, last);
  if (seg == 0) {
    ws->cursor = (u32)first;
    if (!piped) {
      ws->rc_low = 0;
      ws->rc_range = 0xff00000000000000ULL;
      ws->out_len = 0;
    }
    ws->dec_pos = ~0ull;
  }
  constexpr bool paired = MODE >= 2;
  u64 stop;
  if (seg < S) {
    const u64 ns = segment_synchro(seg, S, first, last);
    if (!paired) stop = ns + 1;
    else {
      u64 i = ws->cursor;
      if (i < ns) i += (ns - i + 1) & ~1ull;
      stop = i + 2;
    }
  } else
    stop = last;
  if (stop > last) stop = last;
  FQ_SYNC();
  mt_copy((u64 *)&sm->mt[0][0], (const u64 *)&ws->mt[0][0]);
  for (u32 g = FQ_LANE; g < 4; g += FQ_WAVE) sm->mt_idx[g] = ws->mt_idx[g];
  w.mn[0] = w.mn[1] = w.mn[2] = 0;
  {
    u64 nu = cfg.siv_stats[0], nf = cfg.siv_stats[1];
    w.repm_gate = !((nf ? (double)nu / (double)nf : 0.0) < 7.0);
  }
  w.la[0] = w.la[1] = w.la[2] = 0;
  w.pq_lo[0] = w.pq_lo[1] = 0;
  w.lq_pub[0] = w.lq_pub[1] = 0;
  FQ_SYNC();
  enc_open(w, ws->rc_low, ws->rc_range, ws->out_len, cfg);
  w.avg_code = ws->avg_code; w.avg_letters = ws->avg_letters;
  for (u32 i = 0; i < 4; ++i) w.s_let[i] = ws->s_letters[i];
  w.hidden = ws->hidden_updates;
  w.ctx_letters = 0; w.cor_pos = 0; w.N_run = 0;
  km_reset(w.pm); km_reset(w.sm_); km_reset(w.bm); km_reset(w.pm_u); km_reset(w.sm_u); km_reset(w.bm_u);

  u64 cur = ws->cursor;
  w.pe_n = 0;
  TM_END(w, TX_PROLOG, t_total);
  if (decode) {
    w.din = cfg.din + cfg.din_off[tid];
    w.din_len = cfg.din_off[tid + 1] - cfg.din_off[tid];
    if (ws->dec_pos == ~0ull) rcd_start(w);
    else { w.din_pos = ws->dec_pos; w.dec.low = ws->rc_low; w.dec.range = ws->rc_range; w.dec.buf = ws->dec_buffer; }
    u8 *codes = cfg.dscratch + (u64)tid * 2 * cfg.dcap, *rcodes = codes + cfg.dcap;
    for (u64 i = cur; i < stop && !w.err; i += paired ? 2 : 1) {
      const u64 o0 = cfg.read_off[i], o1 = cfg.read_off[i + 1];
      const u8 *prev_out = nullptr;
      if (i > first) prev_out = cfg.dout + cfg.read_off[i - (paired ? 2 : 1)];
      if (!paired) read_dec(w, codes, cfg.dout + o0, (u32)(o1 - o0), prev_out, true);
      else if (i + 1 < stop) pair_dec(w, codes, rcodes, cfg.dout + o0, (u32)(o1 - o0), cfg.dout + o1, (u32)(cfg.read_off[i + 2] - o1), prev_out);
    }
    ws->dec_pos = w.din_pos;
    ws->dec_buffer = w.dec.buf;
  } else if (heads)
    for (u64 i = cur; i < stop && !w.err; ++i) {
      u64 o0 = cfg.read_off[i], o1 = cfg.read_off[i + 1];
      compress_read_rec(w, cfg.bases + o0, (u32)(o1 - o0), (u32)(i - cur), i + 1 < stop);
    }
  else if (!paired)
    for (u64 i = cur; i < stop && !w.err; ++i) {
      u64 o0 = cfg.read_off[i], o1 = cfg.read_off[i + 1];
      const u8 *prev = nullptr;
      u32 prev_size = 0;
      if (i > first) {
        u64 q0 = cfg.read_off[i - 1];
        prev = cfg.bases + q0;
        prev_size = (u32)(o0 - q0);
      }
      compress_read(w, cfg.bases + o0, (u32)(o1 - o0), prev, prev_size);
    }
  else
    for (u64 i = cur; i + 1 < stop && !w.err; i += 2) {
      u64 o0 = cfg.read_off[i], o1 = cfg.read_off[i + 1], o2 = cfg.read_off[i + 2];
      const u8 *prev = nullptr;
      u32 prev_size = 0;
      if (i > first) {
        u64 q0 = cfg.read_off[i - 2], q1 = cfg.read_off[i - 1];
        prev = cfg.bases + q0;
        prev_size = (u32)(q1 - q0);
      }
      compress_pair(w, cfg.bases + o0, (u32)(o1 - o0), cfg.bases + o1, (u32)(o2 - o1), prev, prev_size);
    }
  if (stop > cur) cur = stop;
  TM_STAMP(cfg, tid, launch, 6);
  lq_flush(w, MAIL_B);
  lq_flush(w, MAIL_S);

  if (piped) {
    FQ_SYNC();
    lds_store_rel(&sm->cq_done, 1u);
    lds_store_rel(&sm->lq_quit, 1u);
  }
  ws->cursor = (u32)cur;
  if (!piped) {
    if (decode) { ws->rc_low = w.dec.low; ws->rc_range = w.dec.range; }
    else {
      enc_close(w);
      ws->rc_low = w.enc.low; ws->rc_range = w.enc.range; ws->out_len = w.enc.len;
    }
    ws->avg_code = w.avg_code; ws->avg_letters = w.avg_letters;
  }
  for (u32 i = 0; i < 4; ++i) ws->s_letters[i] = w.s_let[i];
  ws->hidden_updates = w.hidden;
  TM_END(w, TM_TOTAL, t_total);
  TM_STAMP(cfg, tid, launch, 2);
  TM_TRACE_VAL(cfg, tid, launch, 8, w.tm[CN_SLOW]); TM_TRACE_VAL(cfg, tid, launch, 9, w.tm[CN_ROUGH]);
  TM_TRACE_VAL(cfg, tid, launch, 10, w.tm[CN_DIRTY]); TM_TRACE_VAL(cfg, tid, launch, 11, w.tm[CN_FAST]);
  TM_TRACE_VAL(cfg, tid, launch, 12, w.tm[TM_RRWAIT]); TM_TRACE_VAL(cfg, tid, launch, 13, w.tm[TM_SPEC]);
  TM_TRACE_VAL(cfg, tid, launch, 14, w.tm[CN_GENERIC]); TM_TRACE_VAL(cfg, tid, launch, 15, w.tm[TM_LQ]);
#ifdef FQSX_TIMING
  {
    const u32 xs[16] = {TM_SLOW, TM_SPRE, TM_ROUGH, TM_FINDC, TM_POST, TM_KEYS, TM_READ_HEAD, TM_CQWAIT, TX_QMM, TX_QRUN, TX_PROLOG, TX_CHUNKQ, TX_FLUSH, TM_TOTAL, TX_G_EARLY, TX_OWNSPEC};
    for (u32 x = 0; x < 16; ++x) TM_TRACE_VAL(cfg, tid, launch, 16 + x, w.tm[xs[x]]);
  }
#endif
  if (!piped) {
    for (u32 i = 0; i < ST_N; ++i) ws->stat[i] += w.st[i];
    for (u32 i = 0; i < FQSX_TM_SLOTS && i < 48; ++i) ws->stat[16 + i] += w.tm[i];
  } else if (FQ_LANE == 0) {
    for (u32 i = 0; i < ST_N; ++i) if (w.st[i]) atomic_add64(&ws->stat[i], w.st[i]);
#ifdef FQSX_TIMING
    for (u32 i = 0; i < FQSX_TM_SLOTS && i < 48; ++i) if (w.tm[i]) atomic_add64(&ws->stat[16 + i], w.tm[i]);
#endif
  }
  FQ_SYNC();
  mt_copy((u64 *)&ws->mt[0][0], (const u64 *)&sm->mt[0][0]);
  for (u32 g = FQ_LANE; g < 4; g += FQ_WAVE) ws->mt_idx[g] = sm->mt_idx[g];
  for (u32 k = 0; k < 3; ++k) cfg.mail[k].n[tid] = w.mn[k];
  if (paired) cfg.pe_n[tid] = w.pe_n;
  if (w.err) *cfg.err = w.err;
}

template <class SM>
FQ_DEV void insert_batch(const DevCfg &cfg, SM *sm, const KTab &t, u32 tid, const u64 *keys, u32 n, u32 rng, const Cinc &ci,
                         u64 &nslots, u32 &err) {
  insert_batch_k(cfg, sm, t, tid, FQ_LANE < n ? keys[FQ_LANE] : 0, n, rng, ci, nslots, err);
}
template <class SM>
FQ_DEV void insert_batch_k(const DevCfg &cfg, SM *sm, const KTab &t, u32 tid, u64 mykey, u32 n, u32 rng, const Cinc &ci,
                           u64 &nslots, u32 &err) {
  (void)cfg;
#ifdef FQSX_TIMING
  u64 ib_t[4] = {0, 0, 0, 0}, ib_rounds = 0;
#define IB_MARK(i) do { const u64 now_ = fq_clock(); ib_t[i] += now_ - ib_c; ib_c = now_; } while (0)
  u64 ib_c = fq_clock();
#else
#define IB_MARK(i) ((void)0)
#endif
  u64 *s = t.slots + (u64)tid * t.stride;
  const u64 cm = (1ull << t.cbits) - 1ull;
  const u32 lane = FQ_LANE;
  const u64 v = lane < n ? mykey >> (64 - 2 * t.k) : 0;
  u32 filled = t.filled[tid];
  for (u32 done = 0; done < n;) {
    u64 pos = 0, item = 0;
    bool act = lane >= done && lane < n, found = false;
    if (act) {
      const TabLoc L = t.two ? tab_locate(t, s, v) : tab_locate1(t, s, v);
      pos = L.pos; item = L.item; nslots += L.ns;
      found = item != 0;
    }
    IB_MARK(0);
    u32 lim = n;
#if FQ_WAVE > 1
    FQ_SYNC();
    sm->ib_pos[lane] = act ? pos : ~0ull;
    for (u32 i = lane; i < 256; i += FQ_WAVE) sm->ib_hash[i] = 0;
    FQ_SYNC();
    const u32 hb = (((u32)pos ^ (u32)(pos >> 32)) * 0x9E3779B1u) >> 24;
    if (act) lds_or64(&sm->ib_hash[hb], 1ull << lane);
    FQ_SYNC();
    bool clash = false;
    if (act) {
      u64 cand = sm->ib_hash[hb] & ((1ull << lane) - 1ull);
      while (cand && !clash) {
        const u32 j = ctz64(cand);
        cand &= cand - 1ull;
        clash = sm->ib_pos[j] == pos;
      }
    }
    const u64 cl = wave_ballot(clash);
    if (cl) lim = ctz64(cl);
    act = act && lane < lim;
#else
    lim = done + 1;
#endif
    IB_MARK(1);
    const u32 n_new = popc64(wave_ballot(act && !found));
    if ((u64)(filled + n_new) * 10 >= t.nb * FQSX_BKT * 9) { err = FQSX_ERR_GTAB_FULL; return; }
    const u32 cnt = (u32)(item & cm);
    const bool draw = act && found && cnt > ci.thr && cnt < ci.maxv;
    const u64 dm = wave_ballot(draw);
    u32 r = 0;
    if (dm) {
      const u32 my = popc64(dm & ((1ull << lane) - 1ull)), total = popc64(dm);
      u32 idx = sm->mt_idx[rng];
      const u32 avail = idx >= 624 ? 0 : 624 - idx;
      if (draw && my < avail) r = mt_temper(sm->mt[rng][idx + my]);
      if (total > avail) {
        mt_twist(sm->mt[rng]);
        if (draw && my >= avail) r = mt_temper(sm->mt[rng][my - avail]);
        idx = total - avail;
      } else
        idx += total;
      FQ_SYNC();
      if (lane == 0) sm->mt_idx[rng] = idx;
      FQ_SYNC();
    }
    if (act) {
      if (!found) s[pos] = (v << t.cbits) | 1ull;
      else if (cnt <= ci.thr) { if (cnt < (u32)cm) s[pos] = item + 1; }
      else if (draw && (r % (ci.mult * (cnt - ci.thr)) == 0)) s[pos] = item + 1;
    }
    filled += n_new;
    done = lim;
    if (lane == 0 && done >= n) t.filled[tid] = filled;
    IB_MARK(2);
    FQ_SYNC_MEM();
    IB_MARK(3);
#ifdef FQSX_TIMING
    ++ib_rounds;
#endif
  }
#ifdef FQSX_TIMING
  if (rng < 2 && lane == 0) {
    for (u32 i = 0; i < 4; ++i) atomic_add64(&cfg.ws[tid].stat[16 + 40 + i], ib_t[i]);
    atomic_add64(&cfg.ws[tid].stat[16 + 44], ib_rounds);
    atomic_add64(&cfg.ws[tid].stat[16 + 45], 1);
  }
#endif
#undef IB_MARK
}


FQ_DEV u32 mail_owner(const DevCfg &cfg, u32 kind, u64 x) { return kind == MAIL_P ? p_owner(&cfg, x) : sb_owner(&cfg, x); }
FQ_DEV u32 mail_group(const DevCfg &cfg, u32 kind, u64 x) { return cfg.vmap[mail_owner(cfg, kind, x)]; }
FQ_DEV bool shard_mine(const DevCfg &cfg, u32 w) { return cfg.shard_world <= 1 || w % cfg.shard_world == cfg.shard_rank; }

FQ_DEV void part_count_body(const DevCfg &cfg, u32 kind, u32 blk, u32 *hist ) {
  const Mail &m = cfg.mail[kind];
  const u32 T = cfg.T, s = blk / m.n_tiles, t = blk % m.n_tiles;
  const u32 n = m.n[s], lo = t * FQSX_TILE, hi = n < lo + FQSX_TILE ? n : lo + FQSX_TILE;
  for (u32 d = FQ_LANE; d < 256; d += FQ_WAVE) hist[d] = 0;
  FQ_SYNC();
  for (u32 e = lo + FQ_LANE; e < hi; e += FQ_WAVE) lds_inc32(&hist[mail_group(cfg, kind, m.list[(u64)s * m.cap + e])]);
  FQ_SYNC();
  for (u32 d = FQ_LANE; d < T; d += FQ_WAVE) m.tile_hist[(u64)blk * T + d] = hist[d];
}
FQ_DEV void part_scan_body(const DevCfg &cfg, u32 kind, u32 d) {
  const Mail &m = cfg.mail[kind];
  const u32 T = cfg.T, tiles = T * m.n_tiles;
  u32 run = 0;
  for (u32 base = 0; base < tiles; base += FQ_WAVE) {
    u32 i = base + FQ_LANE;
    u32 v = i < tiles ? m.tile_hist[(u64)i * T + d] : 0;
    u32 ex = wave_excl_scan32(v) + run;
    if (i < tiles) m.tile_hist[(u64)i * T + d] = ex;
    run += wave_sum32(v);
  }
  if (FQ_LANE == 0) m.dst_tot[d] = run;
}
FQ_DEV void part_dstoff_body(const DevCfg &cfg, u32 kind) {
  const Mail &m = cfg.mail[kind];
  u32 run = 0;
  for (u32 base = 0; base < cfg.T; base += FQ_WAVE) {
    const u32 d = base + FQ_LANE;
    const u32 v = d < cfg.T ? m.dst_tot[d] : 0;
    const u32 ex = wave_excl_scan32(v) + run;
    if (d < cfg.T) m.dst_off[d] = ex;
    run += wave_sum32(v);
  }
  if (FQ_LANE == 0) m.dst_off[cfg.T] = run;
}
FQ_DEV void part_scatter_body(const DevCfg &cfg, u32 kind, u32 blk, u32 *cursor , u32 *ld , u64 *gm ,
                              const u32 *doff = nullptr ) {
  const Mail &m = cfg.mail[kind];
  const u32 T = cfg.T, s = blk / m.n_tiles, t = blk % m.n_tiles;
  const u32 n = m.n[s], lo = t * FQSX_TILE, hi = n < lo + FQSX_TILE ? n : lo + FQSX_TILE;
  if (lo >= hi) return;
  for (u32 d = FQ_LANE; d < 256; d += FQ_WAVE) gm[d] = 0;
  for (u32 d = FQ_LANE; d < T; d += FQ_WAVE) cursor[d] = (doff ? doff[d] : m.dst_off[d]) + m.tile_hist[(u64)blk * T + d];
  FQ_SYNC();
  for (u32 base = lo; base < hi; base += FQ_WAVE) {
    const u32 e = base + FQ_LANE, cnt = hi - base < FQ_WAVE ? hi - base : FQ_WAVE;
    u64 x = 0;
    u32 d = 0xffffffffu;
    if (e < hi) {
      x = m.list[(u64)s * m.cap + e];
      d = mail_group(cfg, kind, x);
    }
#if FQ_WAVE > 1
    (void)cnt; (void)ld;
    if (e < hi) lds_or64(&gm[d], 1ull << FQ_LANE);
    FQ_SYNC();
    const u64 mine = e < hi ? gm[d] : 0;
    const u32 rank = popc64(mine & ((1ull << FQ_LANE) - 1ull));
    const u32 later = (mine >> FQ_LANE) >> 1 ? 1u : 0u;
    u32 cur = e < hi ? cursor[d] : 0;
    FQ_SYNC();
    if (e < hi) {
      m.sorted[cur + rank] = x;
      if (later == 0) { cursor[d] = cur + rank + 1; gm[d] = 0; }
    }
    FQ_SYNC();
#else
    ld[FQ_LANE] = d;
    FQ_SYNC();
    u32 rank = 0, later = 0;
    for (u32 q = 0; q < cnt; ++q) {
      u32 dq = ld[q];
      rank += (q < FQ_LANE && dq == d) ? 1u : 0u;
      later += (q > FQ_LANE && dq == d) ? 1u : 0u;
    }
    u32 cur = e < hi ? cursor[d] : 0;
    FQ_SYNC();
    if (e < hi) {
      m.sorted[cur + rank] = x;
      if (later == 0) cursor[d] = cur + rank + 1;
    }
    FQ_SYNC();
#endif
  }
}

FQ_DEV void siv_idx_move(const DevCfg &cfg, u64 idx, u32 from, u32 to) {
  u32 *e = cfg.siv_idx + 4 * (idx >> FQSX_SIV_BLK_LOG);
#ifndef FQSX_EMU
  if (from) atomicSub(&e[from], 1u);
  atomicAdd(&e[to], 1u);
#else
  if (from) e[from] -= 1;
  e[to] += 1;
#endif
}
#ifndef FQSX_INS_WAVES
#define FQSX_INS_WAVES 8u
#endif
#ifndef FQSX_WIN_PER
#define FQSX_WIN_PER 2u
#endif
#define FQSX_INS_WG_PER_CU 2u
#define FQSX_INS_THREADS (FQSX_INS_WAVES * 64u)
#define FQSX_WIN_MAX (FQSX_WIN_PER * FQSX_INS_THREADS)
#define FQSX_WIN_HASH (2u * FQSX_WIN_MAX)
#define FQSX_WIN_MULT_MAX 32u
struct InsWgShared {
  u32 mt[2][624];
  u32 mt_idx[2];
  u64 ib_pos[64];
  u64 ib_hash[256];
  u64 h_tag[FQSX_WIN_HASH];
  u32 h_min[FQSX_WIN_HASH];
  u32 rnd[FQSX_WIN_MAX];
  u32 more[FQSX_WIN_MULT_MAX + 1];
  u32 n_draw[FQSX_WIN_PER][FQSX_INS_WAVES], n_new[FQSX_WIN_PER][FQSX_INS_WAVES];
  u32 in_order;
  u32 filled;
  u32 err;
  u64 acc[2];
};
static_assert(RNG_B == 0 && RNG_S == 1, "InsWgShared.mt holds the streams of the global tables only");
#ifndef FQSX_EMU
static_assert(sizeof(InsWgShared) * FQSX_INS_WG_PER_CU <= 128u * 1024u, "FQSX_INS_WG_PER_CU insert-phase workgroups must fit one CU's LDS with room to spare");

FQ_DEVN u64 tab_claim_new(const KTab t, u64 *s, u64 v) {
  bool claimed = false;
  const u64 *p = tab_find_or_claim(t, s, v, (v << t.cbits) | 1ull, claimed);
  return p && claimed ? (u64)(p - s) : ~0ull;
}

FQ_DEV void insert_windows(const DevCfg &cfg, InsWgShared *sm, const KTab &t, u32 sub, const u64 *keys, u32 n, u32 rng, const Cinc &ci,
                           u32 win, u32 maxmult, u64 &nslots, u32 &err, u32 &n_par, u32 &n_fb) {
  u64 *s = t.slots + (u64)sub * t.stride;
  const u32 cm = (1u << t.cbits) - 1u;
  const u32 tx = FQ_TID, lane = FQ_LANE, wave = FQ_WAVE_ID;
  const u64 below = (1ull << lane) - 1ull;
  win = win < FQSX_WIN_MAX ? win : FQSX_WIN_MAX;
  maxmult = maxmult < 1 ? 1 : maxmult < FQSX_WIN_MULT_MAX ? maxmult : FQSX_WIN_MULT_MAX;
  if (tx == 0) sm->filled = t.filled[sub];
  for (u32 wo = 0; wo < n; wo += win) {
    const u32 wn = n - wo < win ? n - wo : win;
    u32 hs = 128;
    while (hs < 2 * wn) hs <<= 1;
    for (u32 i = tx; i < hs; i += FQSX_INS_THREADS) { sm->h_tag[i] = ~0ull; sm->h_min[i] = ~0u; }
    if (tx <= FQSX_WIN_MULT_MAX) sm->more[tx] = 0;
    if (tx == 0) sm->in_order = 0;
    __syncthreads();
    u64 v[FQSX_WIN_PER], pos[FQSX_WIN_PER], item[FQSX_WIN_PER];
    u32 he[FQSX_WIN_PER], rk[FQSX_WIN_PER];
    bool act[FQSX_WIN_PER], drw[FQSX_WIN_PER];
#pragma unroll
    for (u32 j = 0; j < FQSX_WIN_PER; ++j) {
      const u32 i = j * FQSX_INS_THREADS + tx;
      act[j] = i < wn;
      v[j] = 0; pos[j] = ~0ull; item[j] = 0; he[j] = 0; rk[j] = ~0u; drw[j] = false;
      if (act[j]) {
        v[j] = keys[wo + i] >> (64 - 2 * t.k);
        const TabLoc L = tab_locate_live(t, s, v[j]);
        pos[j] = L.pos; item[j] = L.item; nslots += L.ns;
        u32 h = (u32)((v[j] * 0x9E3779B97F4A7C15ull) >> 40) & (hs - 1);
        for (u32 pr = 0; pr < hs; ++pr) {
          const u64 old = (u64)atomicCAS((unsigned long long *)&sm->h_tag[h], ~0ull, (unsigned long long)v[j]);
          if (old == ~0ull || old == v[j]) break;
          h = (h + 1) & (hs - 1);
        }
        he[j] = h;
      }
    }
    __syncthreads();
    u32 q = 0;
    bool over = false;
    for (;;) {
#pragma unroll
      for (u32 j = 0; j < FQSX_WIN_PER; ++j)
        if (act[j] && rk[j] == ~0u) atomicMin(&sm->h_min[he[j]], ((63u - q) << 16) | (j * FQSX_INS_THREADS + tx));
      __syncthreads();
      bool left = false;
#pragma unroll
      for (u32 j = 0; j < FQSX_WIN_PER; ++j)
        if (act[j] && rk[j] == ~0u) {
          if ((sm->h_min[he[j]] & 0xffffu) == j * FQSX_INS_THREADS + tx) rk[j] = q; else left = true;
        }
      if (left) sm->more[q] = 1;
      __syncthreads();
      if (!sm->more[q]) break;
      if (++q >= maxmult) { over = true; break; }
    }
    bool amb = false;
#pragma unroll
    for (u32 j = 0; j < FQSX_WIN_PER; ++j) {
      const u32 c0 = (u32)item[j] & cm;
      if (act[j] && !over) {
        amb |= insplan_ambiguous(c0, rk[j], ci.thr, ci.maxv);
        drw[j] = insplan_draws(c0, rk[j], ci.thr, ci.maxv);
      }
      const u64 dm = wave_ballot(drw[j]), nm = wave_ballot(act[j] && !over && item[j] == 0 && rk[j] == 0);
      if (lane == 0) { sm->n_draw[j][wave] = popc64(dm); sm->n_new[j][wave] = popc64(nm); }
    }
    if (amb) sm->in_order = 1;
    __syncthreads();
    if (over || sm->in_order) {
      if (wave == 0) {
        __builtin_amdgcn_fence(__ATOMIC_ACQUIRE, "agent");
        u32 e1 = 0;
        insert_keys(cfg, sm, t, sub, keys + wo, wn, rng, ci, nslots, e1);
        FQ_SYNC_MEM();
        if (lane == 0) { sm->filled = t.filled[sub]; if (e1) sm->err = e1; }
      }
      ++n_fb;
      __syncthreads();
      if (sm->err) { err = sm->err; break; }
      continue;
    }
    u32 D = 0, n_new = 0, base[FQSX_WIN_PER];
#pragma unroll
    for (u32 j = 0; j < FQSX_WIN_PER; ++j) base[j] = 0;
#pragma unroll
    for (u32 jj = 0; jj < FQSX_WIN_PER; ++jj)
      for (u32 ww = 0; ww < FQSX_INS_WAVES; ++ww) {
        const u32 c = sm->n_draw[jj][ww];
#pragma unroll
        for (u32 j = 0; j < FQSX_WIN_PER; ++j) base[j] += (jj < j || (jj == j && ww < wave)) ? c : 0u;
        D += c;
        n_new += sm->n_new[jj][ww];
      }
#pragma unroll
    for (u32 j = 0; j < FQSX_WIN_PER; ++j) base[j] += popc64(wave_ballot(drw[j]) & below);
    const u32 filled = sm->filled;
    if ((u64)(filled + n_new) * 10 >= t.nb * FQSX_BKT * 9) { err = FQSX_ERR_GTAB_FULL; break; }
    if (wave == 0 && D) {
      u32 idx = sm->mt_idx[rng];
      for (u32 out = 0; out < D;) {
        if (idx >= 624) { mt_twist(sm->mt[rng]); idx = 0; }
        const u32 take = 624 - idx < D - out ? 624 - idx : D - out;
        for (u32 x = lane; x < take; x += FQ_WAVE) sm->rnd[out + x] = mt_temper(sm->mt[rng][idx + x]);
        FQ_SYNC();
        idx += take; out += take;
      }
      if (lane == 0) sm->mt_idx[rng] = idx;
    }
    bool lost = false;
#pragma unroll
    for (u32 j = 0; j < FQSX_WIN_PER; ++j)
      if (act[j] && item[j] == 0 && rk[j] == 0) {
        pos[j] = tab_claim_new(t, s, v[j]);
        sm->h_tag[he[j]] = pos[j];
        lost |= pos[j] == ~0ull;
      }
    if (lost) sm->err = FQSX_ERR_GTAB_FULL;
    if (tx == 0) t.filled[sub] = filled + n_new;
    __syncthreads();
    if (tx == 0) sm->filled = filled + n_new;
    if (sm->err) { err = sm->err; break; }
    for (u32 r = 0; r <= q; ++r) {
#pragma unroll
      for (u32 j = 0; j < FQSX_WIN_PER; ++j)
        if (act[j] && rk[j] == r && !(item[j] == 0 && r == 0)) {
          u64 *sp = s + (item[j] ? pos[j] : sm->h_tag[he[j]]);
          const u64 cur = r == 0 ? item[j] : __hip_atomic_load(sp, __ATOMIC_RELAXED, __HIP_MEMORY_SCOPE_AGENT);
          if (insplan_adds((u32)cur & cm, drw[j], drw[j] ? sm->rnd[base[j]] : 0u, ci.thr, ci.mult, cm)) *sp = cur + 1;
        }
      FQ_SYNC_MEM();
      __syncthreads();
    }
    ++n_par;
  }
}
#endif

template <class SM>
FQ_DEV void insert_phase_body(const DevCfg &cfg, SM *sm, u32 tid, u32 kind, u32 win, u32 maxmult) {
  WState *ws = cfg.ws + tid;
  const Mail &m = cfg.mail[kind];
  const u32 lo = m.dst_off[tid], hi = m.dst_off[tid + 1];
  if (kind == MAIL_P) {
    u64 nf = 0, nu = 0;
    for (u32 e = lo + FQ_TID; e < hi; e += FQ_NTHREADS) {
      u64 idx = m.sorted[e];
      u64 *wp = cfg.siv + (idx >> 5);
      u32 sh = 2 * (u32)(idx & 31);
      u64 old = *wp;
      for (;;) {
        u64 f = (old >> sh) & 3;
        if (f == 3) break;
        u64 seen = atomic_cas64(wp, old, old + (1ull << sh));
        if (seen == old) {
          nf += f == 0;
          siv_idx_move(cfg, idx, (u32)f, (u32)f + 1);
          if (cfg.siv_part) {
#ifndef FQSX_EMU
            const u32 at = atomicAdd(cfg.p_log_n, 1u);
#else
            const u32 at = (*cfg.p_log_n)++;
#endif
            cfg.p_log[at] = (idx << 4) | (f << 2) | (f + 1);
          }
          break;
        }
        old = seen;
      }
      ++nu;
    }
    nf = wave_sum64(nf);
    nu = wave_sum64(nu);
#ifndef FQSX_EMU
    if (FQ_TID == 0) sm->acc[0] = sm->acc[1] = 0;
    FQ_WG_BARRIER();
    if (FQ_LANE == 0) { atomicAdd((unsigned long long *)&sm->acc[0], (unsigned long long)nf); atomicAdd((unsigned long long *)&sm->acc[1], (unsigned long long)nu); }
    FQ_WG_BARRIER();
    nf = sm->acc[0]; nu = sm->acc[1];
#endif
    if (FQ_TID == 0) {
#ifndef FQSX_EMU
      atomicAdd((unsigned long long *)&cfg.siv_stats[1], (unsigned long long)nf);
      atomicAdd((unsigned long long *)&cfg.siv_stats[0], (unsigned long long)(nu + ws->hidden_updates));
#else
      cfg.siv_stats[1] += nf;
      cfg.siv_stats[0] += nu + ws->hidden_updates;
#endif
      ws->hidden_updates = 0;
      ws->stat[ST_SIV_WORDS] += hi - lo;
    }
    return;
  }
  const KTab &t = kind == MAIL_S ? cfg.g_s : cfg.g_b;
  const u32 rng = kind == MAIL_S ? RNG_S : RNG_B;
  const Cinc ci = kind == MAIL_S ? CINC_S : CINC_B;
  u32 err = 0, n_par = 0, n_fb = 0;
  u64 n_slots = 0;
  for (u32 i = FQ_TID; i < 624; i += FQ_NTHREADS) sm->mt[rng][i] = ws->mt[rng][i];
  if (FQ_TID == 0) { sm->mt_idx[rng] = ws->mt_idx[rng]; sm->err = 0; }
  FQ_WG_BARRIER();
#ifndef FQSX_EMU
  if (win && t.two) insert_windows(cfg, sm, t, tid, m.sorted + lo, hi - lo, rng, ci, win, maxmult, n_slots, err, n_par, n_fb);
  else
#endif
  if (FQ_WAVE_ID == 0) insert_keys(cfg, sm, t, tid, m.sorted + lo, hi - lo, rng, ci, n_slots, err);
  (void)win; (void)maxmult;
  FQ_WG_BARRIER();
  for (u32 i = FQ_TID; i < 624; i += FQ_NTHREADS) ws->mt[rng][i] = sm->mt[rng][i];
  n_slots = wave_sum64(n_slots);
  if (FQ_LANE == 0) {
#ifndef FQSX_EMU
    if (n_slots) atomicAdd((unsigned long long *)&ws->stat[ST_GINS_SLOT], (unsigned long long)n_slots);
#else
    ws->stat[ST_GINS_SLOT] += n_slots;
#endif
    if (err) *cfg.err = err;
  }
  if (FQ_TID == 0) {
    ws->mt_idx[rng] = sm->mt_idx[rng];
#ifndef FQSX_EMU
    atomicAdd((unsigned long long *)&ws->stat[ST_GINS], (unsigned long long)(hi - lo));
    if (n_par) atomicAdd((unsigned long long *)&ws->stat[ST_INS_WIN], (unsigned long long)n_par);
    if (n_fb) atomicAdd((unsigned long long *)&ws->stat[ST_INS_WIN_ORDER], (unsigned long long)n_fb);
#else
    ws->stat[ST_GINS] += hi - lo;
#endif
  }
}

FQ_DEV void finish_block_body(const DevCfg &cfg, u32 tid) {
  WState *ws = cfg.ws + tid;
  u64 low = ws->rc_low, len = ws->out_len;
  u8 *out = cfg.out + (u64)tid * cfg.out_cap;
  for (int i = 0; i < 8; ++i) {
    if (len < cfg.out_cap) out[len] = (u8)(low >> 56); else *cfg.err = FQSX_ERR_OUT_OVERFLOW;
    ++len;
    low <<= 8;
  }
  ws->rc_low = low;
  ws->out_len = len;
}
```

fqsqueezer_amd/csrc/fqsx_layout.h:

```cpp
#pragma once
#include "fqsx_plat.h"

#define FQSX_MAX_T 255
#define FQSX_SIV_BLK_LOG 14u
#define FQSX_SIV_BLK (1u << FQSX_SIV_BLK_LOG)
#define FQSX_NIL 0xffffffffu
#define FQSX_RD_LDS 3072u
#define FQSX_HD 3u
#define FQSX_SPEC 64u
#define FQSX_PQ 512u
#define FQSX_CQ 256u

struct KGeom {
  u32 k, shift;
  u64 mask, kernel_mask;
};

#define FQSX_BKT 4u
struct KTab {
  u64 *slots;
  u64 nb;
  u64 stride;
  u32 *filled;
  u32 k, cbits;
  u32 two, pad_;
};

struct CtxSlot {
  u64 key;
  u32 counter;
  u16 tag;
  u16 total;
  u16 st[5];
  u16 pad[3];
};

#define FQSX_TILE 2048u
struct Mail {
  u64 *list;
  u32 *n;
  u64 *sorted;
  u32 *tile_hist;
  u32 *dst_tot;
  u32 *dst_off;
  u32 cap;
  u32 n_tiles;
};
enum { MAIL_P = 0, MAIL_S = 1, MAIL_B = 2 };

struct PTab {
  u64 *key, *val;
  u64 cap_mask;
  u64 stride;
  u32 *filled;
};

#define SM_FLAGS_N 2u
#define SM_NS_N 2u
#define SM_PSF_N 5u
#define SM_NIB_N 16u
#define SM_BYTE_N 256u
#define SM_OFF_FLAGS 0u
#define SM_OFF_NS (SM_OFF_FLAGS + 256u * (SM_FLAGS_N + 1u))
#define SM_OFF_PSF (SM_OFF_NS + 32u * (SM_NS_N + 1u))
#define SM_OFF_PSNB (SM_OFF_PSF + 65536u * (SM_PSF_N + 1u))
#define SM_OFF_NIB (SM_OFF_PSNB + 65536u * (5u + 1u))
#define SM_OFF_BYTE (SM_OFF_NIB + 68u * (SM_NIB_N + 1u))
#define SM_BYTE_ENTRIES (16u + 16384u)
#define SM_OFF_MPOS (SM_OFF_BYTE + SM_BYTE_ENTRIES * (SM_BYTE_N + 1u))
#define SM_MPOS_ENTRIES 96u
#define SM_OFF_MID (SM_OFF_MPOS + SM_MPOS_ENTRIES * (SM_BYTE_N + 1u))
#define SM_TOTAL_U16 (SM_OFF_MID + (SM_NIB_N + 1u))
#define SM_LAZY_ENTRIES (SM_BYTE_ENTRIES + SM_MPOS_ENTRIES)

struct WState {
  double avg_code, avg_letters;
  u64 ctx_flags, ctx_ps_flags;
  u64 s_letters[4];
  u64 pmer_prev_dir, pmer_prev_rc;
  u32 pmer_prev_cur;
  u32 cursor;
  u64 hidden_updates;
  u64 rc_low, rc_range;
  u64 out_len;
  u64 dec_buffer, dec_pos;
  u32 mt_idx[4];
  alignas(8) u32 mt[4][624];
  u64 stat[64];
};
enum { RNG_B = 0, RNG_S = 1, RNG_LB = 2, RNG_LS = 3 };
enum {
  ST_GPROBE = 0,
  ST_GSLOT,
  ST_LPROBE,
  ST_LSLOT,
  ST_GINS,
  ST_GINS_SLOT,
  ST_SIV_WORDS,
  ST_CTX,
  ST_CODED,
  ST_LINS,
  ST_MAIL,
  ST_BASES,
  ST_SIV_SAVED,
  ST_DEC_REFETCH,
  ST_N,
  ST_INS_WIN = 14,
  ST_INS_WIN_ORDER = 15
};
static_assert(ST_N <= ST_INS_WIN, "WState.stat[14..15] belong to the insert phase, [16..63] to the timing builds");
enum { TM_TOTAL = 0, TM_SPEC, TM_FAST, TM_SLOW, TM_POST, TM_READ_HEAD, TM_LQ, TM_ROUGH, TM_REPM, TM_FINDC,
       CN_FAST, CN_SLOW, CN_CHUNK, CN_DIRTY, CN_ROUGH, CN_REPM,
       CN_EXT, CN_GENERIC, CN_LQFLUSH, TM_RRWAIT , TM_CQWAIT , CN_EARLY, CN_P2, TM_P2,
       TM_CODER_IDLE , TM_SCOUT_WAIT , TM_SPRE,
       TM_CR_S, TM_CR_MID, TM_CR_AVG, TM_CR_RC, TM_KEYS,
       TM_SC_SPEC , TM_SC_EARLY, TM_SC_ROUGH , TM_SC_IDLE , CN_SC_CHUNK, CN_SC_ABORT,
       TM_SP_ROLL , TM_SP_PROBE ,
       TM_N, TM_SP_HIT = 46 , TM_SP_MISS = 47 ,
       TX_QMM = 48 , TX_QRUN , TX_PROLOG ,
       TX_CHUNKQ , TX_FLUSH ,
       TX_G_EARLY , TX_OWNSPEC  };
#ifdef FQSX_TIMING
#define FQSX_TM_SLOTS 56
#else
#define FQSX_TM_SLOTS 1
#endif

struct DevCfg {
  u32 T, mode;
  u32 prefix, pmer, smer, bmer;
  KGeom gp, gs, gb;
  u32 pmer_mod_shift;
  u32 ps_nobytes_n;
  u64 T_magic;
  u32 T_pow2;
  u32 dbg;
  u64 *siv;
  u64 *siv_stats;
  u32 *siv_idx;
  KTab g_s, g_b;
  KTab l_s, l_b;
  CtxSlot *ctx;
  u64 ctx_cap_mask;
  u32 *ctx_filled;
  u16 *small;
  u8 *byte_init;
  WState *ws;
  Mail mail[3];
  PTab g_pe, l_pe;
  u64 *pe_list;
  u32 *pe_n;
  u32 pe_cap;
  u64 *pe_bkt;
  u32 *pe_bkt_n;
  u32 *pe_bkt_cur;
  const u8 *bases;
  const u64 *read_off;
  u8 *out;
  u64 out_cap;
  const u8 *din;
  const u64 *din_off;
  u8 *dout;
  u8 *dscratch;
  u64 dcap;
  u8 *pe_scr;
  u64 pe_scr_cap;
  u32 *err;
  u64 *trace;
  u32 shard_rank, shard_world;
  u32 tab_load_pct;
  u32 whatif;
  u32 sys_scope;
  u32 pe_part;
  u32 siv_part, pad_siv_;
  u64 *p_log;
  u32 *p_log_n;
  const u8 *vmap;
  u32 *shard_cnt;
};

enum {
  FQSX_DBG_SCOUTS_OFF = 1,
  FQSX_DBG_ABANDON = 2,
  FQSX_DBG_RESTART = 4,
  FQSX_DBG_INSERTER_STALL = 8,
};
enum {
  FQSX_ERR_OUT_OVERFLOW = 1,
  FQSX_ERR_GTAB_FULL = 2,
  FQSX_ERR_LTAB_FULL = 3,
  FQSX_ERR_CTX_FULL = 4,
  FQSX_ERR_MAIL_FULL = 5,
  FQSX_ERR_PE_FULL = 6,
  FQSX_ERR_PE_READ_TOO_LONG = 7,
  FQSX_ERR_DECODE = 8,
  FQSX_ERR_PIPE = 9,
};
```

Before: 115.2 Mbases/s.

## Replace count/scan/scatter mail partition with per-source sender kernel and by-source insert

Replaces the three-kernel mail partition (tile count, scan, scatter) with one sender kernel per (kind, source worker). Each sender buckets its own mail list into destination order in its own slice of the sorted buffer, using per-wave LDS histograms, and records per-destination offsets in a new soff matrix. The insert phase then reads keys per source through a prefix array and a binary search over sources. Growth-demand checking moves into the insert kernel itself, which saves kernel launches and the global scan, at the cost of a log(T) search on every key access and extra shared memory.

```diff
diff --git a/fqsqueezer_amd/csrc/fqsx_api.hip b/fqsqueezer_amd/csrc/fqsx_api.hip
--- a/fqsqueezer_amd/csrc/fqsx_api.hip
+++ b/fqsqueezer_amd/csrc/fqsx_api.hip
@@ -27,25 +27,38 @@
 }
 
 FQ_DEV bool phase_skip(const DevCfg &cfg) { return (cfg.err[0] | cfg.err[1]) != 0; }
-FQ_KERNEL_NW(FQSX_INS_THREADS, FQSX_INS_WG_PER_CU * FQSX_INS_WAVES / 4) void k_insert_phase(DevCfg cfg, u64 nb_slots, u64 ns_slots, u32 win, u32 maxmult) {
+FQ_KERNEL_NW(FQSX_INS_THREADS, FQSX_INS_WG_PER_CU * FQSX_INS_WAVES / 4) void k_insert_phase(DevCfg cfg, u64 nb_slots, u64 ns_slots, u32 win, u32 maxmult, u32 by_source, u32 seg1) {
   FQ_SHARED InsWgShared sm;
+  const bool inserts = FQ_BLOCK < 3 * cfg.T;
+  u32 over = 0;
+  if (seg1 && inserts)
+    for (u32 i = FQ_TID; i < 2 * cfg.T; i += FQ_NTHREADS) {
+      const KTab &t = i < cfg.T ? cfg.g_s : cfg.g_b;
+      if (((u64)cfg.demand[2 * cfg.T + 1 + i] + cfg.demand[i]) * 100 > t.nb * FQSX_BKT * cfg.tab_load_pct) over = 2;
+    }
 #ifndef FQSX_EMU
   if (FQ_TID == 0) sm.err = phase_skip(cfg) ? 1u : 0u;
   __syncthreads();
-  const bool skip = sm.err != 0;
+  if (over) atomicOr(&sm.err, over);
   __syncthreads();
-  if (skip) return;
+  const u32 stop = sm.err;
+  __syncthreads();
 #else
-  if (phase_skip(cfg)) return;
+  const u32 stop = (phase_skip(cfg) ? 1u : 0u) | over;
 #endif
-  if (FQ_BLOCK >= 3 * cfg.T) {
+  if (stop & 1) return;
+  if (stop) {
+    if (FQ_TID == 0) { cfg.demand[5 * cfg.T + 1] = seg1; cfg.err[1] = seg1; }
+    return;
+  }
+  if (!inserts) {
     const u64 stride = (u64)(FQ_NBLOCKS - 3 * cfg.T) * FQ_NTHREADS, first = (u64)(FQ_BLOCK - 3 * cfg.T) * FQ_NTHREADS + FQ_TID;
     for (u64 i = first; i < nb_slots; i += stride) cfg.l_b.slots[i] = 0;
     for (u64 i = first; i < ns_slots; i += stride) cfg.l_s.slots[i] = 0;
     for (u64 i = first; i < 2ull * cfg.T; i += stride) cfg.l_s.filled[i] = 0;
     return;
   }
-  insert_phase_body(cfg, &sm, FQ_BLOCK / 3, FQ_BLOCK % 3, win, maxmult);
+  insert_phase_body(cfg, &sm, FQ_BLOCK / 3, FQ_BLOCK % 3, win, maxmult, by_source != 0);
   if (cfg.sys_scope) fq_release_system();
 }
 FQ_KERNEL64 void k_compact_generic(const u8 *out, u64 out_cap, const u64 *lens, u8 *dst) {
@@ -147,6 +160,12 @@
     if (blk == 0) part_dstoff_leader(cfg, kind, demand, seg1);
   }
   part_scatter_body(cfg, kind, blk, cursor, ld, gm, demand ? doff : nullptr);
+}
+static_assert(FQSX_SND_THREADS == 512, "k_part_sender's launch bound");
+FQ_KERNEL512 void k_part_sender(DevCfg cfg) {
+  FQ_SHARED SndShared sm;
+  if (phase_skip(cfg)) return;
+  part_sender_body(cfg, &sm, FQ_BLOCK / cfg.T, FQ_BLOCK % cfg.T);
 }
 FQ_KERNEL64 void k_pe_demand(DevCfg cfg, u32 *demand, u32 seg1) {
   FQ_SHARED InsShared sm;
@@ -541,6 +560,7 @@
   } vm_s, vm_b, vm_pk, vm_pv, vm_siv;
   u32 *d_plog_n;
   u32 ins_win, ins_maxmult;
+  bool part_sender;
   u64 vm_own_bytes;
 };
 
@@ -1005,11 +1025,12 @@
   return FQSX_OK;
 }
 
-int insert_and_clear(fqsx_dna *c) {
+int insert_and_clear(fqsx_dna *c, u32 seg1) {
   const u64 words = (c->cur_need_lb + c->cur_need_ls) * c->T;
   const u64 per = 64ull * FQSX_INS_THREADS;
   const u32 cgrid = (u32)std::min<u64>(2048, (words + per - 1) / per + 1);
-  LAUNCH(c, 1, k_insert_phase, 3 * c->T + cgrid, FQSX_INS_THREADS, c->cfg, c->cur_need_lb * c->T, c->cur_need_ls * c->T, c->ins_win, c->ins_maxmult);
+  LAUNCH(c, 1, k_insert_phase, 3 * c->T + cgrid, FQSX_INS_THREADS, c->cfg, c->cur_need_lb * c->T, c->cur_need_ls * c->T, c->ins_win, c->ins_maxmult,
+         c->part_sender ? 1u : 0u, c->part_sender ? seg1 : 0u);
   return FQSX_OK;
 }
 int grow_for_demand(fqsx_dna *c) {
@@ -1031,10 +1052,15 @@
   const u32 T = c->T;
   int rc;
   if ((rc = d2h_sync(c, c->h_demand.data(), c->d_demand, (4 * T + 1) * sizeof(u32)))) return rc;
+  u32 pairs_done = 0;
+  if (c->paired && c->part_sender) {
+    if ((rc = d2h_sync(c, &pairs_done, c->d_demand + 5 * T + 1, sizeof(u32)))) return rc;
+    if (pairs_done && (rc = dzero(c, c->d_demand + 5 * T + 1, sizeof(u32)))) return rc;
+  }
   const u64 before = c->gs_cap + c->gb_cap + c->gpe_cap;
   if ((rc = grow_for_demand(c))) return rc;
   if ((rc = dzero(c, c->cfg.err + 1, sizeof(u32)))) return rc;
-  if (c->paired) {
+  if (c->paired && !pairs_done) {
     if ((rc = dzero(c, c->cfg.pe_bkt_n, T * sizeof(u32)))) return rc;
     LAUNCH(c, 2, k_pe_demand, T, 64, c->cfg, c->d_demand + 4 * T + 1, 0u);
     std::vector<u32> dem(T), fil(T);
@@ -1045,8 +1071,8 @@
     if (need * 2 > c->gpe_cap && (rc = grow_gpe(c, pow2_at_least(need * 2 + 2)))) return rc;
   }
   if (c->gs_cap + c->gb_cap + c->gpe_cap == before) { g_err = "phase " + std::to_string(seg) + " posted for growth, but no table needs it"; return FQSX_E_DEVICE; }
-  if (c->paired && (rc = pe_insert_and_clear(c))) return rc;
-  return insert_and_clear(c);
+  if (c->paired && !pairs_done && (rc = pe_insert_and_clear(c))) return rc;
+  return insert_and_clear(c, 0);
 }
 int pe_clear_local(fqsx_dna *c) {
   const u32 T = c->T;
@@ -1070,10 +1096,13 @@
   {
     if ((rc = launch_segment(c, decode, n_reads, (u32)S, seg))) return rc;
     const u32 part_grid = T * (cfg.mail[0].n_tiles + cfg.mail[1].n_tiles + cfg.mail[2].n_tiles);
-    LAUNCH(c, 2, k_part_count, part_grid, 64, cfg);
-    LAUNCH(c, 2, k_part_scan, 3 * T, 64, cfg);
+    if (!decode && c->part_sender) LAUNCH(c, 2, k_part_sender, 3 * T, FQSX_SND_THREADS, cfg);
+    else {
+      LAUNCH(c, 2, k_part_count, part_grid, 64, cfg);
+      LAUNCH(c, 2, k_part_scan, 3 * T, 64, cfg);
+      if (!decode) LAUNCH(c, 2, k_part_scatter, part_grid, 64, cfg, seg + 1, c->d_demand);
+    }
     if (!decode) {
-      LAUNCH(c, 2, k_part_scatter, part_grid, 64, cfg, seg + 1, c->d_demand);
       if (c->paired) {
         const u32 bgrid = FQ_GRID((u32)std::min<u64>(1024, ((u64)T * cfg.pe_cap + 255) / 256));
         LAUNCH(c, 2, k_pe_bucket_count, bgrid, 256, cfg);
@@ -1082,7 +1111,7 @@
         LAUNCH(c, 2, k_pe_insert_buckets, T, 64, cfg);
         if ((rc = pe_clear_local(c))) return rc;
       }
-      return insert_and_clear(c);
+      return insert_and_clear(c, seg + 1);
     }
     LAUNCH(c, 2, k_part_dstoff, 3, 64, cfg, c->d_demand, 0u);
     if ((rc = d2h_small_begin(c, c->d_demand, (4 * T + 1) * sizeof(u32)))) return rc;
@@ -1102,7 +1131,7 @@
       if (need * 2 > c->gpe_cap && (rc = grow_gpe(c, pow2_at_least(need * 2 + 2)))) return rc;
       if ((rc = pe_insert_and_clear(c))) return rc;
     }
-    LAUNCH(c, 1, k_insert_phase, 3 * T, FQSX_INS_THREADS, cfg, (u64)0, (u64)0, c->ins_win, c->ins_maxmult);
+    LAUNCH(c, 1, k_insert_phase, 3 * T, FQSX_INS_THREADS, cfg, (u64)0, (u64)0, c->ins_win, c->ins_maxmult, 0u, 0u);
     if ((rc = clear_local_tables(c))) return rc;
   }
   return FQSX_OK;
@@ -1196,6 +1225,8 @@
   if (const char *e = getenv("FQSX_INS_WINDOW")) c->ins_win = (u32)std::min<u64>(FQSX_WIN_MAX, std::max<u64>(1, strtoull(e, nullptr, 10)));
   if (const char *e = getenv("FQSX_INS_MAXMULT")) c->ins_maxmult = (u32)std::min<u64>(FQSX_WIN_MULT_MAX, std::max<u64>(1, strtoull(e, nullptr, 10)));
   if (const char *e = getenv("FQSX_INS_PARALLEL")) if (atoi(e) == 0) c->ins_win = 0;
+  c->part_sender = true;
+  if (const char *e = getenv("FQSX_PART_SENDER")) c->part_sender = atoi(e) != 0;
 #ifdef FQSX_EMU
   c->ins_win = 0;
 #endif
@@ -1261,6 +1292,8 @@
     cfg.mail[k].dst_tot = (u32 *)p;
     if ((rc = dalloc(c, &p, ((u64)T + 1) * sizeof(u32), true))) return rc;
     cfg.mail[k].dst_off = (u32 *)p;
+    if ((rc = dalloc(c, &p, ((u64)T + 1) * T * sizeof(u32), true))) return rc;
+    cfg.mail[k].soff = (u32 *)p;
     if ((rc = mail_alloc(c, k, FQSX_TILE))) return rc;
   }
   c->paired = cfg.mode >= 2;
@@ -1294,7 +1327,7 @@
   cfg.trace = (u64 *)p;
 #endif
   if ((rc = dalloc(c, &p, (5 * (u64)T + 2) * sizeof(u32), true))) return rc;
-  c->d_demand = (u32 *)p;
+  c->d_demand = cfg.demand = (u32 *)p;
   if ((rc = dalloc(c, &p, ((u64)T + 64) * sizeof(u64), true))) return rc;
   c->d_lens = (u64 *)p;
   if ((rc = dalloc(c, &p, (2 * (u64)T + 2) * sizeof(u64), true))) return rc;
@@ -1507,7 +1540,7 @@
   if (tab_over(c, need_s, c->gs_cap) && (rc = grow_global(c, cfg.g_s, c->gs_cap, tab_new_cap(c, need_s)))) return rc;
   if (tab_over(c, need_b, c->gb_cap) && (rc = grow_global(c, cfg.g_b, c->gb_cap, tab_new_cap(c, need_b)))) return rc;
   if ((rc = d2h_sync(c, c->siv_before, cfg.siv_stats, 2 * sizeof(u64)))) return rc;
-  LAUNCH(c, 1, k_insert_phase, 3 * T, FQSX_INS_THREADS, cfg, (u64)0, (u64)0, c->ins_win, c->ins_maxmult);
+  LAUNCH(c, 1, k_insert_phase, 3 * T, FQSX_INS_THREADS, cfg, (u64)0, (u64)0, c->ins_win, c->ins_maxmult, 0u, 0u);
   u64 after[2];
   if ((rc = d2h_sync(c, after, cfg.siv_stats, 2 * sizeof(u64)))) return rc;
   siv_delta[0] = after[0] - c->siv_before[0];
@@ -1641,7 +1674,7 @@
     if (M[MAIL_P]) LAUNCH(c, 2, k_zero_words, (u32)std::min<u64>(REHASH_GRID, (M[MAIL_P] + 255) / 256), 256, cfg.p_log, M[MAIL_P], 0u);
     if ((rc = dzero(c, c->d_plog_n, sizeof(u32)))) return rc;
   }
-  LAUNCH(c, 1, k_insert_phase, 3 * T, FQSX_INS_THREADS, cfg, (u64)0, (u64)0, c->ins_win, c->ins_maxmult);
+  LAUNCH(c, 1, k_insert_phase, 3 * T, FQSX_INS_THREADS, cfg, (u64)0, (u64)0, c->ins_win, c->ins_maxmult, 0u, 0u);
   for (u32 k = 0; k < 3; ++k)
     if (n_items[(u64)k * G + me] && !(k == MAIL_P && cfg.siv_part)) LAUNCH(c, 2, k_shard_collect, REHASH_GRID, 256, cfg, k, c->d_items + off_k[k]);
   if (FW) LAUNCH(c, 2, k_shard_pack2, 1, 64, cfg, (const u64 *)c->d_small, c->d_items + off_siv, c->d_items + off_fill, n_own_max, n_fill);
diff --git a/fqsqueezer_amd/csrc/fqsx_dev.h b/fqsqueezer_amd/csrc/fqsx_dev.h
--- a/fqsqueezer_amd/csrc/fqsx_dev.h
+++ b/fqsqueezer_amd/csrc/fqsx_dev.h
@@ -716,17 +716,37 @@
 template <class SM>
 FQ_DEV void insert_batch_k(const DevCfg &cfg, SM *sm, const KTab &t, u32 sub, u64 mykey, u32 n, u32 rng, const Cinc &ci,
                            u64 &nslots, u32 &err);
-template <class SM>
-FQ_DEV void insert_keys(const DevCfg &cfg, SM *sm, const KTab &t, u32 sub, const u64 *keys, u32 n, u32 rng, const Cinc &ci,
+struct MailKeys {
+  const u64 *p;
+  const u32 *pre;
+  const u32 *at;
+  u32 T, cap, first;
+};
+FQ_DEV u64 key_at(const MailKeys &k, u32 i) {
+  i += k.first;
+  if (!k.pre) return k.p[i];
+  u32 lo = 0, hi = k.T;
+  while (hi - lo > 1) {
+    const u32 mid = (lo + hi) >> 1;
+    if (k.pre[mid] <= i) lo = mid; else hi = mid;
+  }
+  return k.p[(u64)lo * k.cap + k.at[lo] + (i - k.pre[lo])];
+}
+FQ_DEV MailKeys keys_from(MailKeys k, u32 o) { k.first += o; return k; }
+FQ_DEV u64 key_at(const u64 *k, u32 i) { return k[i]; }
+FQ_DEV const u64 *keys_from(const u64 *k, u32 o) { return k + o; }
+
+template <class SM, class K>
+FQ_DEV void insert_keys(const DevCfg &cfg, SM *sm, const KTab &t, u32 sub, const K keys, u32 n, u32 rng, const Cinc &ci,
                         u64 &nslots, u32 &err) {
 #if FQ_WAVE > 1
   const u64 *s = t.slots + (u64)sub * t.stride;
-  u64 nextk = FQ_LANE < n ? keys[FQ_LANE] : 0;
+  u64 nextk = FQ_LANE < n ? key_at(keys, FQ_LANE) : 0;
   for (u32 o = 0; o < n && !err; o += FQ_WAVE) {
     const u64 k = nextk;
     u64 touch = 0;
     if (o + FQ_WAVE + FQ_LANE < n) {
-      nextk = keys[o + FQ_WAVE + FQ_LANE];
+      nextk = key_at(keys, o + FQ_WAVE + FQ_LANE);
       const TabHome th = tab_home(t, nextk >> (64 - 2 * t.k));
       touch = touch_load(&s[(u64)th.a * FQSX_BKT]) ^ touch_load(&s[(u64)th.b * FQSX_BKT]);
     }
@@ -734,7 +754,7 @@
     keep_live(touch);
   }
 #else
-  for (u32 j = 0; j < n && !err; ++j) insert_batch(cfg, sm, t, sub, keys + j, 1, rng, ci, nslots, err);
+  for (u32 j = 0; j < n && !err; ++j) insert_batch_k(cfg, sm, t, sub, key_at(keys, j), 1, rng, ci, nslots, err);
 #endif
 }
 FQ_DEV u32 lq_done_now(Wk &w, u32 qi) { return w.lqh ? lds_load_acq(&w.sm->lq_done[qi]) : w.la[qi ? MAIL_S : MAIL_B]; }
@@ -4134,6 +4154,7 @@
   mt_copy((u64 *)&ws->mt[0][0], (const u64 *)&sm->mt[0][0]);
   for (u32 g = FQ_LANE; g < 4; g += FQ_WAVE) ws->mt_idx[g] = sm->mt_idx[g];
   for (u32 k = 0; k < 3; ++k) cfg.mail[k].n[tid] = w.mn[k];
+  cfg.demand[tid] = cfg.demand[cfg.T + tid] = 0;
   if (paired) cfg.pe_n[tid] = w.pe_n;
   if (w.err) *cfg.err = w.err;
 }
@@ -4330,6 +4351,74 @@
   }
 }
 
+#define FQSX_SND_WAVES 8u
+#define FQSX_SND_THREADS (FQSX_SND_WAVES * 64u)
+struct SndShared {
+  u32 cur[FQSX_SND_WAVES][256];
+  u64 gm[FQSX_SND_WAVES][256];
+};
+FQ_DEV void part_sender_body(const DevCfg &cfg, SndShared *sm, u32 kind, u32 s) {
+  const Mail &m = cfg.mail[kind];
+  const u32 T = cfg.T, n = m.n[s] < m.cap ? m.n[s] : m.cap, wave = FQ_WAVE_ID, n_waves = FQ_NTHREADS / FQ_WAVE;
+  const u64 *list = m.list + (u64)s * m.cap;
+  u64 *dst = m.sorted + (u64)s * m.cap;
+  const u32 per = ((n + n_waves - 1) / n_waves + FQ_WAVE - 1) / FQ_WAVE * FQ_WAVE;
+  const u32 lo = wave * per < n ? wave * per : n, hi = lo + per < n ? lo + per : n;
+  for (u32 d = FQ_TID; d < n_waves * 256; d += FQ_NTHREADS) { sm->cur[d >> 8][d & 255] = 0; sm->gm[d >> 8][d & 255] = 0; }
+  FQ_WG_BARRIER();
+  for (u32 e = lo + FQ_LANE; e < hi; e += FQ_WAVE) lds_inc32(&sm->cur[wave][mail_group(cfg, kind, list[e])]);
+  FQ_WG_BARRIER();
+  if (wave == 0) {
+    u32 *tot = kind == MAIL_P ? nullptr : cfg.demand + (kind == MAIL_S ? 0 : T);
+    u32 run = 0;
+    for (u32 base = 0; base < T; base += FQ_WAVE) {
+      const u32 d = base + FQ_LANE;
+      u32 v = 0;
+      if (d < T)
+        for (u32 w = 0; w < n_waves; ++w) { const u32 c = sm->cur[w][d]; sm->cur[w][d] = v; v += c; }
+      const u32 ex = wave_excl_scan32(v) + run;
+      if (d < T) {
+        for (u32 w = 0; w < n_waves; ++w) sm->cur[w][d] += ex;
+        m.soff[(u64)d * T + s] = ex;
+        if (tot && v) atomic_add32(&tot[d], v);
+      }
+      run += wave_sum32(v);
+    }
+    if (FQ_LANE == 0) {
+      m.soff[(u64)T * T + s] = run;
+      if (tot) cfg.demand[2 * T + 1 + (kind == MAIL_S ? 0 : T) + s] = (kind == MAIL_S ? cfg.g_s : cfg.g_b).filled[s];
+    }
+  }
+  FQ_WG_BARRIER();
+  u32 *cur = sm->cur[wave];
+  u64 *gm = sm->gm[wave];
+  for (u32 base = lo; base < hi; base += FQ_WAVE) {
+    const u32 e = base + FQ_LANE;
+    u64 x = 0;
+    u32 d = 0;
+    if (e < hi) {
+      x = list[e];
+      d = mail_group(cfg, kind, x);
+    }
+#if FQ_WAVE > 1
+    if (e < hi) lds_or64(&gm[d], 1ull << FQ_LANE);
+    FQ_SYNC();
+    const u64 mine = e < hi ? gm[d] : 0;
+    const u32 rank = popc64(mine & ((1ull << FQ_LANE) - 1ull));
+    const bool last = ((mine >> FQ_LANE) >> 1) == 0;
+    const u32 at = e < hi ? cur[d] : 0;
+    FQ_SYNC();
+    if (e < hi) {
+      dst[at + rank] = x;
+      if (last) { cur[d] = at + rank + 1; gm[d] = 0; }
+    }
+    FQ_SYNC();
+#else
+    if (e < hi) dst[cur[d]++] = x;
+#endif
+  }
+}
+
 FQ_DEV void siv_idx_move(const DevCfg &cfg, u64 idx, u32 from, u32 to) {
   u32 *e = cfg.siv_idx + 4 * (idx >> FQSX_SIV_BLK_LOG);
 #ifndef FQSX_EMU
@@ -4365,6 +4454,8 @@
   u32 filled;
   u32 err;
   u64 acc[2];
+  u32 src_pre[FQSX_MAX_T + 2];
+  u32 src_at[FQSX_MAX_T + 1];
 };
 static_assert(RNG_B == 0 && RNG_S == 1, "InsWgShared.mt holds the streams of the global tables only");
 #ifndef FQSX_EMU
@@ -4376,7 +4467,7 @@
   return p && claimed ? (u64)(p - s) : ~0ull;
 }
 
-FQ_DEV void insert_windows(const DevCfg &cfg, InsWgShared *sm, const KTab &t, u32 sub, const u64 *keys, u32 n, u32 rng, const Cinc &ci,
+FQ_DEV void insert_windows(const DevCfg &cfg, InsWgShared *sm, const KTab &t, u32 sub, const MailKeys &keys, u32 n, u32 rng, const Cinc &ci,
                            u32 win, u32 maxmult, u64 &nslots, u32 &err, u32 &n_par, u32 &n_fb) {
   u64 *s = t.slots + (u64)sub * t.stride;
   const u32 cm = (1u << t.cbits) - 1u;
@@ -4402,7 +4493,7 @@
       act[j] = i < wn;
       v[j] = 0; pos[j] = ~0ull; item[j] = 0; he[j] = 0; rk[j] = ~0u; drw[j] = false;
       if (act[j]) {
-        v[j] = keys[wo + i] >> (64 - 2 * t.k);
+        v[j] = key_at(keys, wo + i) >> (64 - 2 * t.k);
         const TabLoc L = tab_locate_live(t, s, v[j]);
         pos[j] = L.pos; item[j] = L.item; nslots += L.ns;
         u32 h = (u32)((v[j] * 0x9E3779B97F4A7C15ull) >> 40) & (hs - 1);
@@ -4450,7 +4541,7 @@
       if (wave == 0) {
         __builtin_amdgcn_fence(__ATOMIC_ACQUIRE, "agent");
         u32 e1 = 0;
-        insert_keys(cfg, sm, t, sub, keys + wo, wn, rng, ci, nslots, e1);
+        insert_keys(cfg, sm, t, sub, keys_from(keys, wo), wn, rng, ci, nslots, e1);
         FQ_SYNC_MEM();
         if (lane == 0) { sm->filled = t.filled[sub]; if (e1) sm->err = e1; }
       }
@@ -4516,14 +4607,35 @@
 #endif
 
 template <class SM>
-FQ_DEV void insert_phase_body(const DevCfg &cfg, SM *sm, u32 tid, u32 kind, u32 win, u32 maxmult) {
+FQ_DEV void insert_phase_body(const DevCfg &cfg, SM *sm, u32 tid, u32 kind, u32 win, u32 maxmult, bool by_source) {
   WState *ws = cfg.ws + tid;
   const Mail &m = cfg.mail[kind];
-  const u32 lo = m.dst_off[tid], hi = m.dst_off[tid + 1];
+  MailKeys keys = {m.sorted, nullptr, nullptr, cfg.T, m.cap, 0};
+  u32 n;
+  if (by_source) {
+    if (FQ_WAVE_ID == 0) {
+      const u32 T = cfg.T;
+      u32 run = 0;
+      for (u32 base = 0; base < T; base += FQ_WAVE) {
+        const u32 s = base + FQ_LANE;
+        const u32 a = s < T ? m.soff[(u64)tid * T + s] : 0, b = s < T ? m.soff[(u64)(tid + 1) * T + s] : 0;
+        const u32 ex = wave_excl_scan32(b - a) + run;
+        if (s < T) { sm->src_at[s] = a; sm->src_pre[s] = ex; }
+        run += wave_sum32(b - a);
+      }
+      if (FQ_LANE == 0) sm->src_pre[T] = run;
+    }
+    FQ_WG_BARRIER();
+    keys.pre = sm->src_pre; keys.at = sm->src_at;
+    n = sm->src_pre[cfg.T];
+  } else {
+    keys.p = m.sorted + m.dst_off[tid];
+    n = m.dst_off[tid + 1] - m.dst_off[tid];
+  }
   if (kind == MAIL_P) {
     u64 nf = 0, nu = 0;
-    for (u32 e = lo + FQ_TID; e < hi; e += FQ_NTHREADS) {
-      u64 idx = m.sorted[e];
+    for (u32 e = FQ_TID; e < n; e += FQ_NTHREADS) {
+      u64 idx = key_at(keys, e);
       u64 *wp = cfg.siv + (idx >> 5);
       u32 sh = 2 * (u32)(idx & 31);
       u64 old = *wp;
@@ -4566,7 +4678,7 @@
       cfg.siv_stats[0] += nu + ws->hidden_updates;
 #endif
       ws->hidden_updates = 0;
-      ws->stat[ST_SIV_WORDS] += hi - lo;
+      ws->stat[ST_SIV_WORDS] += n;
     }
     return;
   }
@@ -4579,10 +4691,10 @@
   if (FQ_TID == 0) { sm->mt_idx[rng] = ws->mt_idx[rng]; sm->err = 0; }
   FQ_WG_BARRIER();
 #ifndef FQSX_EMU
-  if (win && t.two) insert_windows(cfg, sm, t, tid, m.sorted + lo, hi - lo, rng, ci, win, maxmult, n_slots, err, n_par, n_fb);
+  if (win && t.two) insert_windows(cfg, sm, t, tid, keys, n, rng, ci, win, maxmult, n_slots, err, n_par, n_fb);
   else
 #endif
-  if (FQ_WAVE_ID == 0) insert_keys(cfg, sm, t, tid, m.sorted + lo, hi - lo, rng, ci, n_slots, err);
+  if (FQ_WAVE_ID == 0) insert_keys(cfg, sm, t, tid, keys, n, rng, ci, n_slots, err);
   (void)win; (void)maxmult;
   FQ_WG_BARRIER();
   for (u32 i = FQ_TID; i < 624; i += FQ_NTHREADS) ws->mt[rng][i] = sm->mt[rng][i];
@@ -4598,11 +4710,11 @@
   if (FQ_TID == 0) {
     ws->mt_idx[rng] = sm->mt_idx[rng];
 #ifndef FQSX_EMU
-    atomicAdd((unsigned long long *)&ws->stat[ST_GINS], (unsigned long long)(hi - lo));
+    atomicAdd((unsigned long long *)&ws->stat[ST_GINS], (unsigned long long)n);
     if (n_par) atomicAdd((unsigned long long *)&ws->stat[ST_INS_WIN], (unsigned long long)n_par);
     if (n_fb) atomicAdd((unsigned long long *)&ws->stat[ST_INS_WIN_ORDER], (unsigned long long)n_fb);
 #else
-    ws->stat[ST_GINS] += hi - lo;
+    ws->stat[ST_GINS] += n;
 #endif
   }
 }
diff --git a/fqsqueezer_amd/csrc/fqsx_layout.h b/fqsqueezer_amd/csrc/fqsx_layout.h
--- a/fqsqueezer_amd/csrc/fqsx_layout.h
+++ b/fqsqueezer_amd/csrc/fqsx_layout.h
@@ -40,6 +40,7 @@
   u64 *list;
   u32 *n;
   u64 *sorted;
+  u32 *soff;
   u32 *tile_hist;
   u32 *dst_tot;
   u32 *dst_off;
@@ -177,6 +178,7 @@
   u32 *p_log_n;
   const u8 *vmap;
   u32 *shard_cnt;
+  u32 *demand;
 };
 
 enum {
```

Measured after the change: 117.4 Mbases/s, median of 6. 1.9% higher.
